# microsoft/vision-longformer

Hardware: NVIDIA H100
Metric: images/sec ViL-Small 224x224 training (higher is better)
Workload: dtype bf16

## Files before the change

### vision_longformer_b200/csrc/vil_sm90.cuh

```cuda
#pragma once
#include <cuda_bf16.h>
#include <cuda_fp16.h>
#include <stdint.h>

namespace sm90 {

__device__ __forceinline__ uint32_t smem_u32(const void* p) { return (uint32_t)__cvta_generic_to_shared(p); }

__host__ __device__ constexpr int core_off(int r, int c, int K) { return (((r >> 3) * (K >> 3) + (c >> 3)) << 6) + ((r & 7) << 3) + (c & 7); }

__device__ __forceinline__ uint64_t desc(const void* tile, int K, int k16) {
  const uint32_t a = smem_u32(tile) + k16 * 256;
  uint64_t d = (uint64_t)((a >> 4) & 0x3FFF);
  d |= (uint64_t)(128 >> 4) << 16;
  d |= (uint64_t)(((K >> 3) * 128) >> 4) << 32;
  return d;
}

__device__ __forceinline__ void wg_fence() { asm volatile("wgmma.fence.sync.aligned;" ::: "memory"); }
__device__ __forceinline__ void wg_commit() { asm volatile("wgmma.commit_group.sync.aligned;" ::: "memory"); }
__device__ __forceinline__ void wg_wait0() { asm volatile("wgmma.wait_group.sync.aligned 0;" ::: "memory"); }
__device__ __forceinline__ void fence_proxy_async() { asm volatile("fence.proxy.async.shared::cta;" ::: "memory"); }
template <int R>
__device__ __forceinline__ void reg_fence(float (&d)[R]) {
#pragma unroll
  for (int i = 0; i < R; ++i) asm volatile("" : "+f"(d[i])::"memory");
}

__device__ __forceinline__ void wgmma_ss_bf16_n16(float (&d)[8], uint64_t a, uint64_t b, uint32_t acc) {
  asm volatile(
      "{\n\t.reg .pred p;\n\tsetp.ne.b32 p, %10, 0;\n\t"
      "wgmma.mma_async.sync.aligned.m64n16k16.f32.bf16.bf16 {%0,%1,%2,%3,%4,%5,%6,%7}, %8, %9, p, 1, 1, 0, 0;\n\t}"
      : "+f"(d[0]), "+f"(d[1]), "+f"(d[2]), "+f"(d[3]), "+f"(d[4]), "+f"(d[5]), "+f"(d[6]), "+f"(d[7])
      : "l"(a), "l"(b), "r"(acc));
}
__device__ __forceinline__ void wgmma_rs_bf16_n16(float (&d)[8], const uint32_t (&a)[4], uint64_t b, uint32_t acc) {
  asm volatile(
      "{\n\t.reg .pred p;\n\tsetp.ne.b32 p, %13, 0;\n\t"
      "wgmma.mma_async.sync.aligned.m64n16k16.f32.bf16.bf16 {%0,%1,%2,%3,%4,%5,%6,%7}, {%8,%9,%10,%11}, %12, p, 1, 1, 0;\n\t}"
      : "+f"(d[0]), "+f"(d[1]), "+f"(d[2]), "+f"(d[3]), "+f"(d[4]), "+f"(d[5]), "+f"(d[6]), "+f"(d[7])
      : "r"(a[0]), "r"(a[1]), "r"(a[2]), "r"(a[3]), "l"(b), "r"(acc));
}
__device__ __forceinline__ void wgmma_ss_f16_n16(float (&d)[8], uint64_t a, uint64_t b, uint32_t acc) {
  asm volatile(
      "{\n\t.reg .pred p;\n\tsetp.ne.b32 p, %10, 0;\n\t"
      "wgmma.mma_async.sync.aligned.m64n16k16.f32.f16.f16 {%0,%1,%2,%3,%4,%5,%6,%7}, %8, %9, p, 1, 1, 0, 0;\n\t}"
      : "+f"(d[0]), "+f"(d[1]), "+f"(d[2]), "+f"(d[3]), "+f"(d[4]), "+f"(d[5]), "+f"(d[6]), "+f"(d[7])
      : "l"(a), "l"(b), "r"(acc));
}
__device__ __forceinline__ void wgmma_rs_f16_n16(float (&d)[8], const uint32_t (&a)[4], uint64_t b, uint32_t acc) {
  asm volatile(
      "{\n\t.reg .pred p;\n\tsetp.ne.b32 p, %13, 0;\n\t"
      "wgmma.mma_async.sync.aligned.m64n16k16.f32.f16.f16 {%0,%1,%2,%3,%4,%5,%6,%7}, {%8,%9,%10,%11}, %12, p, 1, 1, 0;\n\t}"
      : "+f"(d[0]), "+f"(d[1]), "+f"(d[2]), "+f"(d[3]), "+f"(d[4]), "+f"(d[5]), "+f"(d[6]), "+f"(d[7])
      : "r"(a[0]), "r"(a[1]), "r"(a[2]), "r"(a[3]), "l"(b), "r"(acc));
}
__device__ __forceinline__ void wgmma_ss_bf16_n32(float (&d)[16], uint64_t a, uint64_t b, uint32_t acc) {
  asm volatile(
      "{\n\t.reg .pred p;\n\tsetp.ne.b32 p, %18, 0;\n\t"
      "wgmma.mma_async.sync.aligned.m64n32k16.f32.bf16.bf16 {%0,%1,%2,%3,%4,%5,%6,%7,%8,%9,%10,%11,%12,%13,%14,%15}, %16, %17, p, 1, 1, 0, 0;\n\t}"
      : "+f"(d[0]), "+f"(d[1]), "+f"(d[2]), "+f"(d[3]), "+f"(d[4]), "+f"(d[5]), "+f"(d[6]), "+f"(d[7]), "+f"(d[8]), "+f"(d[9]), "+f"(d[10]), "+f"(d[11]), "+f"(d[12]), "+f"(d[13]), "+f"(d[14]), "+f"(d[15])
      : "l"(a), "l"(b), "r"(acc));
}
__device__ __forceinline__ void wgmma_rs_bf16_n32(float (&d)[16], const uint32_t (&a)[4], uint64_t b, uint32_t acc) {
  asm volatile(
      "{\n\t.reg .pred p;\n\tsetp.ne.b32 p, %21, 0;\n\t"
      "wgmma.mma_async.sync.aligned.m64n32k16.f32.bf16.bf16 {%0,%1,%2,%3,%4,%5,%6,%7,%8,%9,%10,%11,%12,%13,%14,%15}, {%16,%17,%18,%19}, %20, p, 1, 1, 0;\n\t}"
      : "+f"(d[0]), "+f"(d[1]), "+f"(d[2]), "+f"(d[3]), "+f"(d[4]), "+f"(d[5]), "+f"(d[6]), "+f"(d[7]), "+f"(d[8]), "+f"(d[9]), "+f"(d[10]), "+f"(d[11]), "+f"(d[12]), "+f"(d[13]), "+f"(d[14]), "+f"(d[15])
      : "r"(a[0]), "r"(a[1]), "r"(a[2]), "r"(a[3]), "l"(b), "r"(acc));
}
__device__ __forceinline__ void wgmma_ss_f16_n32(float (&d)[16], uint64_t a, uint64_t b, uint32_t acc) {
  asm volatile(
      "{\n\t.reg .pred p;\n\tsetp.ne.b32 p, %18, 0;\n\t"
      "wgmma.mma_async.sync.aligned.m64n32k16.f32.f16.f16 {%0,%1,%2,%3,%4,%5,%6,%7,%8,%9,%10,%11,%12,%13,%14,%15}, %16, %17, p, 1, 1, 0, 0;\n\t}"
      : "+f"(d[0]), "+f"(d[1]), "+f"(d[2]), "+f"(d[3]), "+f"(d[4]), "+f"(d[5]), "+f"(d[6]), "+f"(d[7]), "+f"(d[8]), "+f"(d[9]), "+f"(d[10]), "+f"(d[11]), "+f"(d[12]), "+f"(d[13]), "+f"(d[14]), "+f"(d[15])
      : "l"(a), "l"(b), "r"(acc));
}
__device__ __forceinline__ void wgmma_rs_f16_n32(float (&d)[16], const uint32_t (&a)[4], uint64_t b, uint32_t acc) {
  asm volatile(
      "{\n\t.reg .pred p;\n\tsetp.ne.b32 p, %21, 0;\n\t"
      "wgmma.mma_async.sync.aligned.m64n32k16.f32.f16.f16 {%0,%1,%2,%3,%4,%5,%6,%7,%8,%9,%10,%11,%12,%13,%14,%15}, {%16,%17,%18,%19}, %20, p, 1, 1, 0;\n\t}"
      : "+f"(d[0]), "+f"(d[1]), "+f"(d[2]), "+f"(d[3]), "+f"(d[4]), "+f"(d[5]), "+f"(d[6]), "+f"(d[7]), "+f"(d[8]), "+f"(d[9]), "+f"(d[10]), "+f"(d[11]), "+f"(d[12]), "+f"(d[13]), "+f"(d[14]), "+f"(d[15])
      : "r"(a[0]), "r"(a[1]), "r"(a[2]), "r"(a[3]), "l"(b), "r"(acc));
}
__device__ __forceinline__ void wgmma_ss_bf16_n64(float (&d)[32], uint64_t a, uint64_t b, uint32_t acc) {
  asm volatile(
      "{\n\t.reg .pred p;\n\tsetp.ne.b32 p, %34, 0;\n\t"
      "wgmma.mma_async.sync.aligned.m64n64k16.f32.bf16.bf16 {%0,%1,%2,%3,%4,%5,%6,%7,%8,%9,%10,%11,%12,%13,%14,%15,%16,%17,%18,%19,%20,%21,%22,%23,%24,%25,%26,%27,%28,%29,%30,%31}, %32, %33, p, 1, 1, 0, 0;\n\t}"
      : "+f"(d[0]), "+f"(d[1]), "+f"(d[2]), "+f"(d[3]), "+f"(d[4]), "+f"(d[5]), "+f"(d[6]), "+f"(d[7]), "+f"(d[8]), "+f"(d[9]), "+f"(d[10]), "+f"(d[11]), "+f"(d[12]), "+f"(d[13]), "+f"(d[14]), "+f"(d[15]), "+f"(d[16]), "+f"(d[17]), "+f"(d[18]), "+f"(d[19]), "+f"(d[20]), "+f"(d[21]), "+f"(d[22]), "+f"(d[23]), "+f"(d[24]), "+f"(d[25]), "+f"(d[26]), "+f"(d[27]), "+f"(d[28]), "+f"(d[29]), "+f"(d[30]), "+f"(d[31])
      : "l"(a), "l"(b), "r"(acc));
}
__device__ __forceinline__ void wgmma_rs_bf16_n64(float (&d)[32], const uint32_t (&a)[4], uint64_t b, uint32_t acc) {
  asm volatile(
      "{\n\t.reg .pred p;\n\tsetp.ne.b32 p, %37, 0;\n\t"
      "wgmma.mma_async.sync.aligned.m64n64k16.f32.bf16.bf16 {%0,%1,%2,%3,%4,%5,%6,%7,%8,%9,%10,%11,%12,%13,%14,%15,%16,%17,%18,%19,%20,%21,%22,%23,%24,%25,%26,%27,%28,%29,%30,%31}, {%32,%33,%34,%35}, %36, p, 1, 1, 0;\n\t}"
      : "+f"(d[0]), "+f"(d[1]), "+f"(d[2]), "+f"(d[3]), "+f"(d[4]), "+f"(d[5]), "+f"(d[6]), "+f"(d[7]), "+f"(d[8]), "+f"(d[9]), "+f"(d[10]), "+f"(d[11]), "+f"(d[12]), "+f"(d[13]), "+f"(d[14]), "+f"(d[15]), "+f"(d[16]), "+f"(d[17]), "+f"(d[18]), "+f"(d[19]), "+f"(d[20]), "+f"(d[21]), "+f"(d[22]), "+f"(d[23]), "+f"(d[24]), "+f"(d[25]), "+f"(d[26]), "+f"(d[27]), "+f"(d[28]), "+f"(d[29]), "+f"(d[30]), "+f"(d[31])
      : "r"(a[0]), "r"(a[1]), "r"(a[2]), "r"(a[3]), "l"(b), "r"(acc));
}
__device__ __forceinline__ void wgmma_ss_f16_n64(float (&d)[32], uint64_t a, uint64_t b, uint32_t acc) {
  asm volatile(
      "{\n\t.reg .pred p;\n\tsetp.ne.b32 p, %34, 0;\n\t"
      "wgmma.mma_async.sync.aligned.m64n64k16.f32.f16.f16 {%0,%1,%2,%3,%4,%5,%6,%7,%8,%9,%10,%11,%12,%13,%14,%15,%16,%17,%18,%19,%20,%21,%22,%23,%24,%25,%26,%27,%28,%29,%30,%31}, %32, %33, p, 1, 1, 0, 0;\n\t}"
      : "+f"(d[0]), "+f"(d[1]), "+f"(d[2]), "+f"(d[3]), "+f"(d[4]), "+f"(d[5]), "+f"(d[6]), "+f"(d[7]), "+f"(d[8]), "+f"(d[9]), "+f"(d[10]), "+f"(d[11]), "+f"(d[12]), "+f"(d[13]), "+f"(d[14]), "+f"(d[15]), "+f"(d[16]), "+f"(d[17]), "+f"(d[18]), "+f"(d[19]), "+f"(d[20]), "+f"(d[21]), "+f"(d[22]), "+f"(d[23]), "+f"(d[24]), "+f"(d[25]), "+f"(d[26]), "+f"(d[27]), "+f"(d[28]), "+f"(d[29]), "+f"(d[30]), "+f"(d[31])
      : "l"(a), "l"(b), "r"(acc));
}
__device__ __forceinline__ void wgmma_rs_f16_n64(float (&d)[32], const uint32_t (&a)[4], uint64_t b, uint32_t acc) {
  asm volatile(
      "{\n\t.reg .pred p;\n\tsetp.ne.b32 p, %37, 0;\n\t"
      "wgmma.mma_async.sync.aligned.m64n64k16.f32.f16.f16 {%0,%1,%2,%3,%4,%5,%6,%7,%8,%9,%10,%11,%12,%13,%14,%15,%16,%17,%18,%19,%20,%21,%22,%23,%24,%25,%26,%27,%28,%29,%30,%31}, {%32,%33,%34,%35}, %36, p, 1, 1, 0;\n\t}"
      : "+f"(d[0]), "+f"(d[1]), "+f"(d[2]), "+f"(d[3]), "+f"(d[4]), "+f"(d[5]), "+f"(d[6]), "+f"(d[7]), "+f"(d[8]), "+f"(d[9]), "+f"(d[10]), "+f"(d[11]), "+f"(d[12]), "+f"(d[13]), "+f"(d[14]), "+f"(d[15]), "+f"(d[16]), "+f"(d[17]), "+f"(d[18]), "+f"(d[19]), "+f"(d[20]), "+f"(d[21]), "+f"(d[22]), "+f"(d[23]), "+f"(d[24]), "+f"(d[25]), "+f"(d[26]), "+f"(d[27]), "+f"(d[28]), "+f"(d[29]), "+f"(d[30]), "+f"(d[31])
      : "r"(a[0]), "r"(a[1]), "r"(a[2]), "r"(a[3]), "l"(b), "r"(acc));
}

template <typename T, int N> struct Wg;
#define VIL_WG(T, TN, N)                                                                                          \
  template <> struct Wg<T, N> {                                                                                   \
    static __device__ __forceinline__ void ss(float (&d)[N / 2], uint64_t a, uint64_t b, uint32_t acc) { wgmma_ss_##TN##_n##N(d, a, b, acc); } \
    static __device__ __forceinline__ void rs(float (&d)[N / 2], const uint32_t (&a)[4], uint64_t b, uint32_t acc) { wgmma_rs_##TN##_n##N(d, a, b, acc); } \
  };
VIL_WG(__nv_bfloat16, bf16, 16)
VIL_WG(__nv_bfloat16, bf16, 32)
VIL_WG(__nv_bfloat16, bf16, 64)
VIL_WG(__half, f16, 16)
VIL_WG(__half, f16, 32)
VIL_WG(__half, f16, 64)
#undef VIL_WG

template <typename T> __device__ __forceinline__ uint32_t pack2(float x, float y);
template <> __device__ __forceinline__ uint32_t pack2<__nv_bfloat16>(float x, float y) {
  __nv_bfloat162 v = __floats2bfloat162_rn(x, y);
  return *reinterpret_cast<uint32_t*>(&v);
}
template <> __device__ __forceinline__ uint32_t pack2<__half>(float x, float y) {
  __half2 v = __floats2half2_rn(x, y);
  return *reinterpret_cast<uint32_t*>(&v);
}

}
```

### vision_longformer_b200/csrc/vil_wgmma.cu

```cuda
#include <cstdio>
#include "vil_host.cuh"
#include "vil_wgmma.cuh"

namespace vil {
namespace {

int head_tile(int D) { return D <= 16 ? 16 : D <= 32 ? 32 : 64; }
int table_floats(const Geo& g) { return g.has_bias ? (4 * g.w - 1) * (4 * g.w - 1) : 0; }

template <typename K>
int set_smem(K kernel, size_t bytes) {
  if (bytes > 227 * 1024) return shared_fail(VIL_E_UNSUPPORTED, "configuration needs more than 227 KB of shared memory");
  cudaError_t e = cudaFuncSetAttribute(kernel, cudaFuncAttributeMaxDynamicSharedMemorySize, (int)bytes);
  if (e != cudaSuccess) return shared_fail(VIL_E_CUDA, cudaGetErrorString(e));
  return VIL_OK;
}

const char* why_not(const VilAttnParams* p, const Geo& g) {
  if (p->dtype != VIL_BF16 && p->dtype != VIL_F16) return "dtype is fp32 (wgmma operands are bf16 / fp16)";
  if (g.D > 64) return "head dim > 64";
  if (wg::DkvSmem<64>::total(table_floats(g)) > 227 * 1024) return "bias table does not fit in shared memory";
  return nullptr;
}

long long blocks(const Geo& g) { return (long long)g.B * g.H * g.mx * g.my * g.npc; }

template <typename T, int HD, typename TO, bool DROP>
int forward_t(const VilAttnParams* p, const Geo& g, cudaStream_t s) {
  int rc;
  if (!(p->skip_mask & 2)) {
    const size_t sm = wg::FwdSmem<HD>::total(table_floats(g));
    if ((rc = set_smem(wg::wg_fwd_local<T, HD, TO, DROP>, sm))) return rc;
    wg::wg_fwd_local<T, HD, TO, DROP><<<(unsigned)blocks(g), wg::kThreads, sm, s>>>(g, t4(p->q), t4(p->k), t4(p->v), t4(p->o), p->lse,
                                                                            p->bias_table, p->g2l);
    count_launch();
    if ((rc = launch_check("wgmma_fwd_local"))) return rc;
  }
  if (g.g > 0 && !(p->skip_mask & 1)) return simt_global_fwd(p, g, s);
  return VIL_OK;
}

template <typename T, int HD, typename TO, bool DROP>
int backward_t(const VilAttnParams* p, const Geo& g, cudaStream_t s) {
  int rc;
  if (!(p->skip_mask & 8) && (rc = simt_delta(p, g, s))) return rc;
  float* delta = static_cast<float*>(p->workspace);
  const int tabn = table_floats(g);
  if (!(p->skip_mask & 2)) {
    const size_t sm = wg::DqSmem<HD>::total(tabn);
    if ((rc = set_smem(wg::wg_bwd_dq<T, HD, TO, DROP>, sm))) return rc;
    wg::wg_bwd_dq<T, HD, TO, DROP><<<(unsigned)blocks(g), wg::kThreads, sm, s>>>(g, t4(p->q), t4(p->k), t4(p->v), t4(p->d_o), t4(p->dq),
                                                                         p->lse, delta, p->bias_table, p->g2l, p->d_bias_table);
    count_launch();
    if ((rc = launch_check("wgmma_bwd_dq"))) return rc;
  }
  if (!(p->skip_mask & 4)) {
    const size_t sm = wg::DkvSmem<HD>::total(tabn, DROP);
    if ((rc = set_smem(wg::wg_bwd_dkv<T, HD, TO, DROP>, sm))) return rc;
    wg::wg_bwd_dkv<T, HD, TO, DROP><<<(unsigned)blocks(g), wg::kThreads, sm, s>>>(g, t4(p->q), t4(p->k), t4(p->v), t4(p->d_o), t4(p->dk),
                                                                          t4(p->dv), p->lse, delta, p->bias_table);
    count_launch();
    if ((rc = launch_check("wgmma_bwd_dkv"))) return rc;
  }
  if (g.g > 0 && !(p->skip_mask & 1)) return simt_global_bwd(p, g, s, g.N);
  return VIL_OK;
}

template <typename T, typename TO, bool DROP>
int dispatch_hd_drop(const VilAttnParams* p, const Geo& g, cudaStream_t s, bool bwd) {
  switch (head_tile(g.D)) {
    case 16: return bwd ? backward_t<T, 16, TO, DROP>(p, g, s) : forward_t<T, 16, TO, DROP>(p, g, s);
    case 32: return bwd ? backward_t<T, 32, TO, DROP>(p, g, s) : forward_t<T, 32, TO, DROP>(p, g, s);
    default: return bwd ? backward_t<T, 64, TO, DROP>(p, g, s) : forward_t<T, 64, TO, DROP>(p, g, s);
  }
}

template <typename T, typename TO>
int dispatch_hd(const VilAttnParams* p, const Geo& g, cudaStream_t s, bool bwd) {
  return g.drop_p > 0.f ? dispatch_hd_drop<T, TO, true>(p, g, s, bwd) : dispatch_hd_drop<T, TO, false>(p, g, s, bwd);
}

int run(const VilAttnParams* p, const Geo& g, cudaStream_t s, bool bwd) {
  note_kernel(bwd ? "wgmma_bwd" : "wgmma_fwd");
  if (p->dtype == VIL_BF16)
    return out_f32(p) ? dispatch_hd<__nv_bfloat16, float>(p, g, s, bwd) : dispatch_hd<__nv_bfloat16, __nv_bfloat16>(p, g, s, bwd);
  return out_f32(p) ? dispatch_hd<__half, float>(p, g, s, bwd) : dispatch_hd<__half, __half>(p, g, s, bwd);
}

}

const char* tc_why_not(const VilAttnParams* p, const Geo& g, bool) {
  const char* w = why_not(p, g);
  return w ? w : "supported";
}
int tc_supported(const VilAttnParams* p, const Geo& g, bool) { return why_not(p, g) == nullptr; }
int tc_forward(const VilAttnParams* p, const Geo& g, cudaStream_t s) { return run(p, g, s, false); }
int tc_backward(const VilAttnParams* p, const Geo& g, cudaStream_t s) { return run(p, g, s, true); }

}
```

### vision_longformer_b200/csrc/vil_wgmma.cuh

```cuda
#pragma once
#include "vil_common.cuh"
#include "vil_sm90.cuh"

namespace vil {
namespace wg {

constexpr int kThreads = 128;

struct Cta { int b, h, R, C, piece; };

__device__ __forceinline__ Cta decode(const Geo& g, int bid) {
  Cta c;
  c.piece = bid % g.npc; bid /= g.npc;
  c.C = bid % g.my; bid /= g.my;
  c.R = bid % g.mx; bid /= g.mx;
  c.h = bid % g.H;
  c.b = bid / g.H;
  return c;
}

__device__ __forceinline__ int acc_row(int i) { return ((threadIdx.x >> 5) << 4) + ((threadIdx.x & 31) >> 2) + (((i >> 1) & 1) << 3); }
__device__ __forceinline__ int acc_col(int i) { return ((i >> 2) << 3) + ((threadIdx.x & 3) << 1) + (i & 1); }

template <typename T, int HD>
__device__ __forceinline__ void stage_half_row(T* tile, T* tile_t, const float (&x)[HD / 2], int row, int half) {
  constexpr int HH = HD / 2;
#pragma unroll
  for (int g8 = 0; g8 < HH / 8; ++g8) {
    uint4 u;
    u.x = sm90::pack2<T>(x[g8 * 8 + 0], x[g8 * 8 + 1]);
    u.y = sm90::pack2<T>(x[g8 * 8 + 2], x[g8 * 8 + 3]);
    u.z = sm90::pack2<T>(x[g8 * 8 + 4], x[g8 * 8 + 5]);
    u.w = sm90::pack2<T>(x[g8 * 8 + 6], x[g8 * 8 + 7]);
    *reinterpret_cast<uint4*>(tile + sm90::core_off(row, half * HH + g8 * 8, HD)) = u;
  }
  if (tile_t != nullptr) {
#pragma unroll
    for (int i = 0; i < HH; ++i) tile_t[sm90::core_off(half * HH + i, row, 64)] = ElemTraits<T>::from_f(x[i]);
  }
}

template <typename T>
__device__ __forceinline__ void to_a_frag(const float (&s)[32], int kk, uint32_t (&a)[4]) {
  a[0] = sm90::pack2<T>(s[8 * kk + 0], s[8 * kk + 1]);
  a[1] = sm90::pack2<T>(s[8 * kk + 2], s[8 * kk + 3]);
  a[2] = sm90::pack2<T>(s[8 * kk + 4], s[8 * kk + 5]);
  a[3] = sm90::pack2<T>(s[8 * kk + 6], s[8 * kk + 7]);
}

template <typename TO, int HD>
__device__ __forceinline__ void store_rows(const float (&acc)[HD / 2], int e, TO* row, int D, float mul) {
  const int c0 = (threadIdx.x & 3) << 1;
#pragma unroll
  for (int j = 0; j < HD / 8; ++j) {
    const int col = 8 * j + c0;
    if (col < D) row[col] = ElemTraits<TO>::from_f(acc[4 * j + 2 * e] * mul);
    if (col + 1 < D) row[col + 1] = ElemTraits<TO>::from_f(acc[4 * j + 2 * e + 1] * mul);
  }
}

__device__ __forceinline__ void drop_key_piece(float (&x)[32], const Geo& geo, const uint32_t (&row)[2], int cbase, uint32_t sid,
                                               float mul) {
  uint32_t keep = 0;
#pragma unroll 1
  for (int i = 0; i < 32; i += 2) {
    bool k0, k1;
    drop_keep2(geo, (i & 2) ? row[1] : row[0], (uint32_t)(cbase + acc_col(i)), sid, k0, k1);
    keep |= ((uint32_t)k0 | ((uint32_t)k1 << 1)) << i;
  }
#pragma unroll
  for (int i = 0; i < 32; ++i) x[i] = (keep >> i) & 1u ? x[i] * mul : 0.f;
}

__device__ __forceinline__ void drop_rows(const Geo& geo, int R, int C, int piece, uint32_t (&row)[2]) {
#pragma unroll
  for (int e = 0; e < 2; ++e) {
    const int l = piece * 64 + acc_row(2 * e);
    row[e] = (uint32_t)((R * geo.w + l / geo.w) * geo.ny + C * geo.w + l % geo.w);
  }
}

struct Visit {
  int r, c;
  int dR, dC;
  int cut;
  int oi;
};

__device__ __forceinline__ int visit_list(const Geo& geo, int R, int C, int sgn, Visit* vl) {
  int n = 0;
  for (int oi = 0; oi < geo.noffs; ++oi) {
    const int dR = geo.offR[oi], dC = geo.offC[oi];
    int r = R + sgn * dR, c = C + sgn * dC;
    if (geo.exact == -1) { r = (r + geo.mx) % geo.mx; c = (c + geo.my) % geo.my; }
    else if (r < 0 || r >= geo.mx || c < 0 || c >= geo.my) continue;
    const int qR = sgn > 0 ? R : r, qC = sgn > 0 ? C : c;
    if (threadIdx.x == 0) vl[n] = Visit{r, c, dR, dC, (qR + dR == geo.mx - 1) | ((qC + dC == geo.my - 1) << 1), oi};
    ++n;
  }
  return n;
}

__device__ __forceinline__ int drop_col_base(const Geo& geo, const Visit* vl, int ngp, int pi) {
  if (pi < ngp) return pi * 64;
  const int vi = (pi - ngp) / geo.npc;
  return geo.g + vl[vi].oi * geo.w2 + (pi - ngp - vi * geo.npc) * 64;
}

__device__ __forceinline__ void chunk_key(const Geo& geo, const Visit& v, int lk, long long& tok, bool& ok, int& vr, int& vc) {
  const int w = geo.w, kr = lk / w, kc = lk - kr * w;
  const int ar = v.r * w + kr, ac = v.c * w + kc;
  const bool real = (ar < geo.nx) && (ac < geo.ny);
  if (geo.exact == -1)
    ok = !(((v.cut & 1) && (kr >= w - geo.padx)) || ((v.cut & 2) && (kc >= w - geo.pady)));
  else
    ok = real;
  tok = (ok && real) ? geo.g + (long long)ar * geo.ny + ac : -1;
  vr = v.dR * w + kr; vc = v.dC * w + kc;
}

__device__ __forceinline__ void key_slot(const Geo& geo, const Visit* vl, int ngp, int pi, int slot, int& gk, long long& tok,
                                         bool& ok, int& vr, int& vc) {
  gk = -1; tok = -1; ok = false; vr = 0; vc = 0;
  if (pi < ngp) {
    const int t = pi * 64 + slot;
    if (t < geo.g) { gk = t; tok = t; ok = true; }
    return;
  }
  const int vi = (pi - ngp) / geo.npc, lk = (pi - ngp - vi * geo.npc) * 64 + slot;
  if (lk < geo.w2) chunk_key(geo, vl[vi], lk, tok, ok, vr, vc);
}

struct KeyCols {
  float* bias;
  int* tix;
  short* kr;
  short* kc;
};
struct QRows {
  int qr[2], qc[2];
  bool ok[2];
};

__device__ __forceinline__ QRows query_rows(const Geo& geo, int R, int C, int piece) {
  QRows q;
  const int w = geo.w;
#pragma unroll
  for (int e = 0; e < 2; ++e) {
    const int l = piece * 64 + acc_row(2 * e);
    const bool in = l < geo.w2;
    q.qr[e] = in ? l / w : 0; q.qc[e] = in ? l % w : 0;
    q.ok[e] = in && (R * w + q.qr[e] < geo.nx) && (C * w + q.qc[e] < geo.ny);
  }
  return q;
}

__device__ __forceinline__ void stage_key_cols(const Geo& geo, const KeyCols& kc, int h, const float* __restrict__ g2l, int gk,
                                               bool ok, int vr, int vc) {
  const int slot = threadIdx.x >> 1;
  float bias = ok ? 0.f : -INFINITY;
  if (gk >= 0 && geo.has_bias) bias = g2l[((long long)geo.H + h) * geo.g + gk];
  kc.bias[slot] = bias;
  kc.tix[slot] = vr * (4 * geo.w - 1) + vc;
  kc.kr[slot] = (short)vr;
  kc.kc[slot] = (short)vc;
}

__device__ __forceinline__ void row_tix(const Geo& geo, const QRows& q, int (&tb)[2]) {
  const int w = geo.w, tw = 4 * w - 1;
  tb[0] = (q.qr[0] + 2 * w - 1) * tw + q.qc[0] + 2 * w - 1;
  tb[1] = (q.qr[1] + 2 * w - 1) * tw + q.qc[1] + 2 * w - 1;
}

template <bool RPE, bool WIN>
__device__ __forceinline__ float key_score(const Geo& geo, const KeyCols& kc, const float* tab, const QRows& q, const int (&tb)[2],
                                           int e, int j, int gl, float s, int& bidx) {
  float bias = kc.bias[j];
  bidx = -1;
  if (RPE && j >= gl) { bidx = tb[e] - kc.tix[j]; bias += tab[bidx]; }
  if (WIN && (abs(q.qr[e] - kc.kr[j]) > geo.w || abs(q.qc[e] - kc.kc[j]) > geo.w)) return -INFINITY;
  return fmaf(geo.scale, s, bias);
}

__device__ __forceinline__ int key_epilogue(const Geo& geo) { return (geo.has_bias ? 2 : 0) | (geo.exact == 1 ? 1 : 0); }

template <bool RPE, bool WIN>
__device__ __forceinline__ void fwd_scores(float (&s)[32], float (&mx)[2], const Geo& geo, const KeyCols& kc, const float* tab,
                                           const QRows& q, int gl) {
  int tb[2] = {0, 0};
  if (RPE) row_tix(geo, q, tb);
#pragma unroll
  for (int i = 0; i < 32; ++i) {
    const int e = (i >> 1) & 1;
    int bidx;
    s[i] = key_score<RPE, WIN>(geo, kc, tab, q, tb, e, acc_col(i), gl, s[i], bidx);
    mx[e] = fmaxf(mx[e], s[i]);
  }
}

template <bool RPE, bool WIN>
__device__ __forceinline__ void dq_scores(float (&s)[32], const float (&dp)[32], const Geo& geo, const KeyCols& kc,
                                          const float* tab, const QRows& q, int gl, const float (&lse_r)[2],
                                          const float (&del_r)[2], float* __restrict__ d_table, int h) {
  int tb[2] = {0, 0};
  if (RPE) row_tix(geo, q, tb);
#pragma unroll
  for (int i = 0; i < 32; ++i) {
    const int e = (i >> 1) & 1;
    int bidx;
    const float val = key_score<RPE, WIN>(geo, kc, tab, q, tb, e, acc_col(i), gl, s[i], bidx);
    const float ds = __expf(val - lse_r[e]) * (dp[i] - del_r[e]);
    if (RPE && d_table != nullptr && bidx >= 0 && q.ok[e] && val != -INFINITY)
      atomicAdd(d_table + (long long)bidx * geo.H + h, ds);
    s[i] = ds;
  }
}

constexpr size_t kKeyMeta = 64 * (4 + 4 + 2 + 2) + 9 * sizeof(Visit);
constexpr size_t kQueryMeta = 64 * (4 + 4 + 4 + 2 + 2 + 1) + 9 * sizeof(Visit);

__device__ __forceinline__ KeyCols key_cols(float* base, Visit*& vl) {
  KeyCols kc;
  kc.bias = base;
  kc.tix = reinterpret_cast<int*>(kc.bias + 64);
  vl = reinterpret_cast<Visit*>(kc.tix + 64);
  kc.kr = reinterpret_cast<short*>(vl + 9);
  kc.kc = kc.kr + 64;
  return kc;
}

template <int HD> struct FwdSmem {
  static constexpr size_t tiles = 3 * 64 * HD * 2;
  static size_t total(int tabn) { return (tiles + (size_t)tabn * 4 + kKeyMeta + 15) & ~size_t(15); }
};
template <int HD> struct DqSmem {
  static constexpr size_t tiles = 5 * 64 * HD * 2;
  static size_t total(int tabn) { return (tiles + (size_t)tabn * 4 + kKeyMeta + 15) & ~size_t(15); }
};
template <int HD> struct DkvSmem {
  static constexpr size_t tiles = 6 * 64 * HD * 2;
  static size_t total(int tabn, bool drop = false) {
    return (tiles + (size_t)tabn * 4 + kQueryMeta + (drop ? 64 * sizeof(int) : 0) + 15) & ~size_t(15);
  }
};

template <typename T, int HD, typename TO, bool DROP = false>
__global__ void __launch_bounds__(kThreads, HD <= 32 ? 5 : 3)
wg_fwd_local(Geo geo, T4 q, T4 k, T4 v, T4 o, float* __restrict__ lse, const float* __restrict__ table,
             const float* __restrict__ g2l) {
  constexpr int HH = HD / 2;
  using W64 = sm90::Wg<T, 64>;
  using WHD = sm90::Wg<T, HD>;
  extern __shared__ __align__(128) unsigned char smem_raw[];
  T* Qs = reinterpret_cast<T*>(smem_raw);
  T* Ks = Qs + 64 * HD;
  T* Vt = Ks + 64 * HD;
  float* tab = reinterpret_cast<float*>(Vt + 64 * HD);
  const int tabn = geo.has_bias ? (4 * geo.w - 1) * (4 * geo.w - 1) : 0;
  Visit* vl;
  const KeyCols kcol = key_cols(tab + tabn, vl);

  const Cta cid = decode(geo, blockIdx.x);
  const int b = cid.b, h = cid.h, R = cid.R, C = cid.C;
  const int tid = threadIdx.x, slot = tid >> 1, half = tid & 1;
  const int w = geo.w, D = geo.D;
  for (int i = tid; i < tabn; i += kThreads) tab[i] = table[(long long)i * geo.H + h];
  {
    const int l = cid.piece * 64 + slot;
    const int r = R * w + l / w, c = C * w + l % w;
    float x[HH];
#pragma unroll
    for (int i = 0; i < HH; ++i) x[i] = 0.f;
    if (l < geo.w2 && r < geo.nx && c < geo.ny) load_seg<T, HH>(row_ptr<T>(q, b, h, (long long)r * geo.ny + c), half * HH, D, x);
    stage_half_row<T, HD>(Qs, nullptr, x, slot, half);
  }
  float m[2] = {-INFINITY, -INFINITY}, lsum[2] = {0.f, 0.f};
  float oacc[HH];
#pragma unroll
  for (int i = 0; i < HH; ++i) oacc[i] = 0.f;

  const int ngp = (geo.g + 63) / 64, npieces = ngp + visit_list(geo, R, C, 1, vl) * geo.npc;
  const int epi = key_epilogue(geo);
  for (int pi = 0; pi < npieces; ++pi) {
    __syncthreads();
    {
      int gk, vr, vc;
      long long tok;
      bool ok;
      key_slot(geo, vl, ngp, pi, slot, gk, tok, ok, vr, vc);
      float kk[HH], vv[HH];
#pragma unroll
      for (int i = 0; i < HH; ++i) { kk[i] = 0.f; vv[i] = 0.f; }
      if (tok >= 0) {
        load_seg<T, HH>(row_ptr<T>(k, b, h, tok), half * HH, D, kk);
        load_seg<T, HH>(row_ptr<T>(v, b, h, tok), half * HH, D, vv);
      }
      stage_half_row<T, HD>(Ks, nullptr, kk, slot, half);
#pragma unroll
      for (int i = 0; i < HH; ++i) Vt[sm90::core_off(half * HH + i, slot, 64)] = ElemTraits<T>::from_f(vv[i]);
      if (half == 0) stage_key_cols(geo, kcol, h, g2l, gk, ok, vr, vc);
    }
    sm90::fence_proxy_async();
    __syncthreads();
    float s[32];
    sm90::wg_fence();
#pragma unroll
    for (int kk = 0; kk < HD / 16; ++kk) W64::ss(s, sm90::desc(Qs, HD, kk), sm90::desc(Ks, HD, kk), kk > 0);
    sm90::wg_commit();
    sm90::wg_wait0();
    sm90::reg_fence(s);
    float mx[2] = {-INFINITY, -INFINITY};
    const int gl = geo.g - pi * 64;
    switch (epi) {
      case 0: fwd_scores<false, false>(s, mx, geo, kcol, tab, query_rows(geo, R, C, cid.piece), gl); break;
      case 1: fwd_scores<false, true>(s, mx, geo, kcol, tab, query_rows(geo, R, C, cid.piece), gl); break;
      case 2: fwd_scores<true, false>(s, mx, geo, kcol, tab, query_rows(geo, R, C, cid.piece), gl); break;
      default: fwd_scores<true, true>(s, mx, geo, kcol, tab, query_rows(geo, R, C, cid.piece), gl); break;
    }
    float corr[2];
#pragma unroll
    for (int e = 0; e < 2; ++e) {
      mx[e] = fmaxf(mx[e], __shfl_xor_sync(0xffffffffu, mx[e], 1));
      mx[e] = fmaxf(mx[e], __shfl_xor_sync(0xffffffffu, mx[e], 2));
      const float mn = fmaxf(m[e], mx[e]);
      corr[e] = (mn == -INFINITY) ? 1.f : __expf(m[e] - mn);
      m[e] = mn;
      lsum[e] *= corr[e];
    }
#pragma unroll
    for (int i = 0; i < 32; ++i) {
      const int e = (i >> 1) & 1;
      const float p = (m[e] == -INFINITY) ? 0.f : __expf(s[i] - m[e]);
      s[i] = p;
      lsum[e] += p;
    }
#pragma unroll
    for (int i = 0; i < HH; ++i) oacc[i] *= corr[(i >> 1) & 1];
    if constexpr (DROP) {
      uint32_t drow[2];
      drop_rows(geo, R, C, cid.piece, drow);
      drop_key_piece(s, geo, drow, drop_col_base(geo, vl, ngp, pi), 2u * (uint32_t)(b * geo.H + h), 1.f);
    }
    uint32_t a[4][4];
#pragma unroll
    for (int kk = 0; kk < 4; ++kk) to_a_frag<T>(s, kk, a[kk]);
    sm90::wg_fence();
#pragma unroll
    for (int kk = 0; kk < 4; ++kk) WHD::rs(oacc, a[kk], sm90::desc(Vt, 64, kk), 1);
    sm90::wg_commit();
    sm90::wg_wait0();
    sm90::reg_fence(oacc);
  }
  const QRows qrow = query_rows(geo, R, C, cid.piece);
#pragma unroll
  for (int e = 0; e < 2; ++e) {
    lsum[e] += __shfl_xor_sync(0xffffffffu, lsum[e], 1);
    lsum[e] += __shfl_xor_sync(0xffffffffu, lsum[e], 2);
    if (!qrow.ok[e]) continue;
    const long long tokq = (long long)(R * w + qrow.qr[e]) * geo.ny + (C * w + qrow.qc[e]);
    const float inv = lsum[e] > 0.f ? 1.f / lsum[e] : 0.f;
    store_rows<TO, HD>(oacc, e, row_ptr_w<TO>(o, b, h, tokq), D, DROP ? inv * geo.drop_scale : inv);
    if ((tid & 3) == 0) lse[((long long)b * geo.H + h) * geo.Nloc + tokq] = m[e] + logf(lsum[e]);
  }
}

template <typename T, int HD, typename TO, bool DROP = false>
__global__ void __launch_bounds__(kThreads)
wg_bwd_dq(Geo geo, T4 q, T4 k, T4 v, T4 d_o, T4 dq, const float* __restrict__ lse, const float* __restrict__ delta,
          const float* __restrict__ table, const float* __restrict__ g2l, float* __restrict__ d_table) {
  constexpr int HH = HD / 2;
  using W64 = sm90::Wg<T, 64>;
  using WHD = sm90::Wg<T, HD>;
  extern __shared__ __align__(128) unsigned char smem_raw[];
  T* Qs = reinterpret_cast<T*>(smem_raw);
  T* Gs = Qs + 64 * HD;
  T* Ks = Gs + 64 * HD;
  T* Vs = Ks + 64 * HD;
  T* Kt = Vs + 64 * HD;
  float* tab = reinterpret_cast<float*>(Kt + 64 * HD);
  const int tabn = geo.has_bias ? (4 * geo.w - 1) * (4 * geo.w - 1) : 0;
  Visit* vl;
  const KeyCols kcol = key_cols(tab + tabn, vl);

  const Cta cid = decode(geo, blockIdx.x);
  const int b = cid.b, h = cid.h, R = cid.R, C = cid.C;
  const int tid = threadIdx.x, slot = tid >> 1, half = tid & 1;
  const int w = geo.w, D = geo.D;
  const long long bh = (long long)b * geo.H + h;
  for (int i = tid; i < tabn; i += kThreads) tab[i] = table[(long long)i * geo.H + h];
  {
    const int l = cid.piece * 64 + slot;
    const int r = R * w + l / w, c = C * w + l % w;
    float x[HH], y[HH];
#pragma unroll
    for (int i = 0; i < HH; ++i) { x[i] = 0.f; y[i] = 0.f; }
    if (l < geo.w2 && r < geo.nx && c < geo.ny) {
      load_seg<T, HH>(row_ptr<T>(q, b, h, (long long)r * geo.ny + c), half * HH, D, x);
      load_seg<T, HH>(row_ptr<T>(d_o, b, h, (long long)r * geo.ny + c), half * HH, D, y);
    }
    stage_half_row<T, HD>(Qs, nullptr, x, slot, half);
    stage_half_row<T, HD>(Gs, nullptr, y, slot, half);
  }
  const QRows qrow = query_rows(geo, R, C, cid.piece);
  float lse_r[2], del_r[2];
#pragma unroll
  for (int e = 0; e < 2; ++e) {
    lse_r[e] = INFINITY; del_r[e] = 0.f;
    if (qrow.ok[e]) {
      const long long tokq = (long long)(R * w + qrow.qr[e]) * geo.ny + (C * w + qrow.qc[e]);
      lse_r[e] = lse[bh * geo.Nloc + tokq];
      del_r[e] = delta[bh * geo.Nloc + tokq];
    }
  }
  float dqacc[HH];
#pragma unroll
  for (int i = 0; i < HH; ++i) dqacc[i] = 0.f;

  const int ngp = (geo.g + 63) / 64, npieces = ngp + visit_list(geo, R, C, 1, vl) * geo.npc;
  const int epi = key_epilogue(geo);
  for (int pi = 0; pi < npieces; ++pi) {
    __syncthreads();
    {
      int gk, vr, vc;
      long long tok;
      bool ok;
      key_slot(geo, vl, ngp, pi, slot, gk, tok, ok, vr, vc);
      float kk[HH], vv[HH];
#pragma unroll
      for (int i = 0; i < HH; ++i) { kk[i] = 0.f; vv[i] = 0.f; }
      if (tok >= 0) {
        load_seg<T, HH>(row_ptr<T>(k, b, h, tok), half * HH, D, kk);
        load_seg<T, HH>(row_ptr<T>(v, b, h, tok), half * HH, D, vv);
      }
      stage_half_row<T, HD>(Ks, Kt, kk, slot, half);
      stage_half_row<T, HD>(Vs, nullptr, vv, slot, half);
      if (half == 0) stage_key_cols(geo, kcol, h, g2l, gk, ok, vr, vc);
    }
    sm90::fence_proxy_async();
    __syncthreads();
    float s[32], dp[32];
    sm90::wg_fence();
#pragma unroll
    for (int kk = 0; kk < HD / 16; ++kk) W64::ss(s, sm90::desc(Qs, HD, kk), sm90::desc(Ks, HD, kk), kk > 0);
#pragma unroll
    for (int kk = 0; kk < HD / 16; ++kk) W64::ss(dp, sm90::desc(Gs, HD, kk), sm90::desc(Vs, HD, kk), kk > 0);
    sm90::wg_commit();
    sm90::wg_wait0();
    sm90::reg_fence(s);
    sm90::reg_fence(dp);
    const int gl = geo.g - pi * 64;
    if constexpr (DROP) {
      uint32_t drow[2];
      drop_rows(geo, R, C, cid.piece, drow);
      drop_key_piece(dp, geo, drow, drop_col_base(geo, vl, ngp, pi), 2u * (uint32_t)(b * geo.H + h), geo.drop_scale);
    }
    switch (epi) {
      case 0: dq_scores<false, false>(s, dp, geo, kcol, tab, qrow, gl, lse_r, del_r, d_table, h); break;
      case 1: dq_scores<false, true>(s, dp, geo, kcol, tab, qrow, gl, lse_r, del_r, d_table, h); break;
      case 2: dq_scores<true, false>(s, dp, geo, kcol, tab, qrow, gl, lse_r, del_r, d_table, h); break;
      default: dq_scores<true, true>(s, dp, geo, kcol, tab, qrow, gl, lse_r, del_r, d_table, h); break;
    }
    uint32_t a[4][4];
#pragma unroll
    for (int kk = 0; kk < 4; ++kk) to_a_frag<T>(s, kk, a[kk]);
    sm90::wg_fence();
#pragma unroll
    for (int kk = 0; kk < 4; ++kk) WHD::rs(dqacc, a[kk], sm90::desc(Kt, 64, kk), 1);
    sm90::wg_commit();
    sm90::wg_wait0();
    sm90::reg_fence(dqacc);
  }
#pragma unroll
  for (int e = 0; e < 2; ++e) {
    if (!qrow.ok[e]) continue;
    const long long tokq = (long long)(R * w + qrow.qr[e]) * geo.ny + (C * w + qrow.qc[e]);
    store_rows<TO, HD>(dqacc, e, row_ptr_w<TO>(dq, b, h, tokq), D, geo.scale);
  }
}


struct QueryCols {
  float* lse;
  float* del;
  int* tix;
  short* qr;
  short* qc;
  unsigned char* cut;
  int* tok;
};
struct KRows {
  int kr[2], kc[2], tb[2];
  int cut[2];
  bool real[2];
};

__device__ __forceinline__ QueryCols query_cols(float* base, Visit*& vl) {
  QueryCols qc;
  qc.lse = base;
  qc.del = qc.lse + 64;
  qc.tix = reinterpret_cast<int*>(qc.del + 64);
  vl = reinterpret_cast<Visit*>(qc.tix + 64);
  qc.qr = reinterpret_cast<short*>(vl + 9);
  qc.qc = qc.qr + 64;
  qc.cut = reinterpret_cast<unsigned char*>(qc.qc + 64);
  qc.tok = reinterpret_cast<int*>(qc.cut + 64);
  return qc;
}

__device__ __forceinline__ int query_epilogue(const Geo& geo) {
  return (geo.has_bias ? 3 : 0) + (geo.exact == 1 ? 1 : geo.exact == -1 ? 2 : 0);
}

template <bool RPE, int MASK>
__device__ __forceinline__ void dkv_probs(float (&s)[32], float (&dp)[32], const Geo& geo, const QueryCols& qc, const float* tab,
                                          const KRows& kr) {
#pragma unroll
  for (int i = 0; i < 32; ++i) {
    const int e = (i >> 1) & 1, j = acc_col(i);
    float x = fmaf(geo.scale, s[i], RPE ? tab[qc.tix[j] - kr.tb[e]] : 0.f) - qc.lse[j];
    if (MASK == 1 && (abs(qc.qr[j] - kr.kr[e]) > geo.w || abs(qc.qc[j] - kr.kc[e]) > geo.w)) x = -INFINITY;
    if (MASK == 2 && (qc.cut[j] & kr.cut[e])) x = -INFINITY;
    const float p = __expf(x);
    s[i] = p;
    dp[i] = p * (dp[i] - qc.del[j]);
  }
}

template <typename T, int HD, typename TO, bool DROP = false>
__global__ void __launch_bounds__(kThreads)
wg_bwd_dkv(Geo geo, T4 q, T4 k, T4 v, T4 d_o, T4 dk, T4 dv, const float* __restrict__ lse, const float* __restrict__ delta,
           const float* __restrict__ table) {
  constexpr int HH = HD / 2;
  using W64 = sm90::Wg<T, 64>;
  using WHD = sm90::Wg<T, HD>;
  extern __shared__ __align__(128) unsigned char smem_raw[];
  T* Ks = reinterpret_cast<T*>(smem_raw);
  T* Vs = Ks + 64 * HD;
  T* Qs = Vs + 64 * HD;
  T* Gs = Qs + 64 * HD;
  T* Qt = Gs + 64 * HD;
  T* Gt = Qt + 64 * HD;
  float* tab = reinterpret_cast<float*>(Gt + 64 * HD);
  const int tw = 4 * geo.w - 1;
  const int tabn = geo.has_bias ? tw * tw : 0;
  Visit* vl;
  const QueryCols qcol = query_cols(tab + tabn, vl);

  const Cta cid = decode(geo, blockIdx.x);
  const int b = cid.b, h = cid.h, KR = cid.R, KC = cid.C;
  const int tid = threadIdx.x, slot = tid >> 1, half = tid & 1;
  const int w = geo.w, D = geo.D;
  const long long bh = (long long)b * geo.H + h;
  for (int i = tid; i < tabn; i += kThreads) tab[i] = table[(long long)i * geo.H + h];
  {
    const int lk = cid.piece * 64 + slot;
    const int ar = KR * w + lk / w, ac = KC * w + lk % w;
    float x[HH], y[HH];
#pragma unroll
    for (int i = 0; i < HH; ++i) { x[i] = 0.f; y[i] = 0.f; }
    if (lk < geo.w2 && ar < geo.nx && ac < geo.ny) {
      const long long tokk = geo.g + (long long)ar * geo.ny + ac;
      load_seg<T, HH>(row_ptr<T>(k, b, h, tokk), half * HH, D, x);
      load_seg<T, HH>(row_ptr<T>(v, b, h, tokk), half * HH, D, y);
    }
    stage_half_row<T, HD>(Ks, nullptr, x, slot, half);
    stage_half_row<T, HD>(Vs, nullptr, y, slot, half);
  }
  KRows krow;
#pragma unroll
  for (int e = 0; e < 2; ++e) {
    const int lk = cid.piece * 64 + acc_row(2 * e);
    const bool in = lk < geo.w2;
    krow.kr[e] = in ? lk / w : 0; krow.kc[e] = in ? lk % w : 0;
    krow.real[e] = in && (KR * w + krow.kr[e] < geo.nx) && (KC * w + krow.kc[e] < geo.ny);
    krow.tb[e] = krow.kr[e] * tw + krow.kc[e] - (2 * w - 1) * (tw + 1);
    krow.cut[e] = (krow.kr[e] >= w - geo.padx) | ((krow.kc[e] >= w - geo.pady) << 1);
  }
  float dkacc[HH], dvacc[HH];
#pragma unroll
  for (int i = 0; i < HH; ++i) { dkacc[i] = 0.f; dvacc[i] = 0.f; }

  const int npieces = visit_list(geo, KR, KC, -1, vl) * geo.npc;
  const int epi = query_epilogue(geo);
  for (int qp = 0; qp < npieces; ++qp) {
    __syncthreads();
    {
      const int vi = qp / geo.npc, l = (qp - vi * geo.npc) * 64 + slot;
      bool qv = false;
      long long tq = 0;
      int qa = 0, qb = 0, cut = 0;
      if (l < geo.w2) {
        const int qrr = l / w, qcc = l - qrr * w;
        const Visit vq = vl[vi];
        const int r = vq.r * w + qrr, c = vq.c * w + qcc;
        qv = (r < geo.nx) && (c < geo.ny);
        tq = (long long)r * geo.ny + c;
        qa = qrr - vq.dR * w; qb = qcc - vq.dC * w; cut = vq.cut;
      }
      float x[HH], y[HH];
#pragma unroll
      for (int i = 0; i < HH; ++i) { x[i] = 0.f; y[i] = 0.f; }
      if (qv) {
        load_seg<T, HH>(row_ptr<T>(q, b, h, tq), half * HH, D, x);
        load_seg<T, HH>(row_ptr<T>(d_o, b, h, tq), half * HH, D, y);
      }
      stage_half_row<T, HD>(Qs, Qt, x, slot, half);
      stage_half_row<T, HD>(Gs, Gt, y, slot, half);
      if (half == 0) {
        qcol.lse[slot] = qv ? lse[bh * geo.Nloc + tq] : INFINITY;
        qcol.del[slot] = qv ? delta[bh * geo.Nloc + tq] : 0.f;
        qcol.tix[slot] = qa * tw + qb;
        qcol.qr[slot] = (short)qa; qcol.qc[slot] = (short)qb;
        qcol.cut[slot] = (unsigned char)cut;
        if (DROP) qcol.tok[slot] = (int)tq;
      }
    }
    sm90::fence_proxy_async();
    __syncthreads();
    float s[32], dp[32];
    sm90::wg_fence();
#pragma unroll
    for (int kk = 0; kk < HD / 16; ++kk) W64::ss(s, sm90::desc(Ks, HD, kk), sm90::desc(Qs, HD, kk), kk > 0);
#pragma unroll
    for (int kk = 0; kk < HD / 16; ++kk) W64::ss(dp, sm90::desc(Vs, HD, kk), sm90::desc(Gs, HD, kk), kk > 0);
    sm90::wg_commit();
    sm90::wg_wait0();
    sm90::reg_fence(s);
    sm90::reg_fence(dp);
    uint32_t keep = 0;
    if constexpr (DROP) {
      const int vi = qp / geo.npc;
      const uint32_t c0 = (uint32_t)(geo.g + vl[vi].oi * geo.w2 + cid.piece * 64), sid = 2u * (uint32_t)(b * geo.H + h);
#pragma unroll 1
      for (int i = 0; i < 32; ++i)
        keep |= (uint32_t)drop_keep(geo, (uint32_t)qcol.tok[acc_col(i)], c0 + (uint32_t)acc_row(i), sid) << i;
#pragma unroll
      for (int i = 0; i < 32; ++i) dp[i] = (keep >> i) & 1u ? dp[i] * geo.drop_scale : 0.f;
    }
    switch (epi) {
      case 0: dkv_probs<false, 0>(s, dp, geo, qcol, tab, krow); break;
      case 1: dkv_probs<false, 1>(s, dp, geo, qcol, tab, krow); break;
      case 2: dkv_probs<false, 2>(s, dp, geo, qcol, tab, krow); break;
      case 3: dkv_probs<true, 0>(s, dp, geo, qcol, tab, krow); break;
      case 4: dkv_probs<true, 1>(s, dp, geo, qcol, tab, krow); break;
      default: dkv_probs<true, 2>(s, dp, geo, qcol, tab, krow); break;
    }
    if constexpr (DROP) {
#pragma unroll
      for (int i = 0; i < 32; ++i) s[i] = (keep >> i) & 1u ? s[i] * geo.drop_scale : 0.f;
    }
    uint32_t ap[4][4], ad[4][4];
#pragma unroll
    for (int kk = 0; kk < 4; ++kk) { to_a_frag<T>(s, kk, ap[kk]); to_a_frag<T>(dp, kk, ad[kk]); }
    sm90::wg_fence();
#pragma unroll
    for (int kk = 0; kk < 4; ++kk) WHD::rs(dvacc, ap[kk], sm90::desc(Gt, 64, kk), 1);
#pragma unroll
    for (int kk = 0; kk < 4; ++kk) WHD::rs(dkacc, ad[kk], sm90::desc(Qt, 64, kk), 1);
    sm90::wg_commit();
    sm90::wg_wait0();
    sm90::reg_fence(dvacc);
    sm90::reg_fence(dkacc);
  }
#pragma unroll
  for (int e = 0; e < 2; ++e) {
    if (!krow.real[e]) continue;
    const long long tokk = geo.g + (long long)(KR * w + krow.kr[e]) * geo.ny + (KC * w + krow.kc[e]);
    store_rows<TO, HD>(dkacc, e, row_ptr_w<TO>(dk, b, h, tokk), D, geo.scale);
    store_rows<TO, HD>(dvacc, e, row_ptr_w<TO>(dv, b, h, tokk), D, 1.f);
  }
}

}
}
```

Before: 3635.

## Pipeline K/V and Q/dO staging with cp.async ring buffers in attention kernels

Replaces the synchronous register load, convert and store of each key/value or query/grad-output piece with a three-stage cp.async ring buffer. The next pieces' global loads now overlap the current piece's wgmma work. The explicitly transposed Q/dO tiles are dropped; the second GEMMs read the same tiles through transposed (MN-major) wgmma descriptors. The cost is more shared memory per CTA, which lowers occupancy, plus a new 16-byte alignment requirement that sends misaligned inputs to the fallback path.

```diff
diff --git a/vision_longformer_b200/csrc/vil_sm90.cuh b/vision_longformer_b200/csrc/vil_sm90.cuh
--- a/vision_longformer_b200/csrc/vil_sm90.cuh
+++ b/vision_longformer_b200/csrc/vil_sm90.cuh
@@ -9,13 +9,25 @@
 
 __host__ __device__ constexpr int core_off(int r, int c, int K) { return (((r >> 3) * (K >> 3) + (c >> 3)) << 6) + ((r & 7) << 3) + (c & 7); }
 
+__device__ __forceinline__ uint64_t make_desc(uint32_t addr, uint32_t lbo, uint32_t sbo) {
+  return (uint64_t)((addr >> 4) & 0x3FFF) | (uint64_t)(lbo >> 4) << 16 | (uint64_t)(sbo >> 4) << 32;
+}
 __device__ __forceinline__ uint64_t desc(const void* tile, int K, int k16) {
-  const uint32_t a = smem_u32(tile) + k16 * 256;
-  uint64_t d = (uint64_t)((a >> 4) & 0x3FFF);
-  d |= (uint64_t)(128 >> 4) << 16;
-  d |= (uint64_t)(((K >> 3) * 128) >> 4) << 32;
-  return d;
+  return make_desc(smem_u32(tile) + k16 * 256, 128, (K >> 3) * 128);
 }
+__device__ __forceinline__ uint64_t desc_mn(const void* tile, int N, int k16) {
+  return make_desc(smem_u32(tile) + k16 * N * 32, N * 16, 128);
+}
+
+__device__ __forceinline__ void cp_async16(void* dst, const void* src, int n) {
+  asm volatile("cp.async.cg.shared.global [%0], [%1], 16, %2;" ::"r"(smem_u32(dst)), "l"(src), "r"(n) : "memory");
+}
+__device__ __forceinline__ void cp_async4(void* dst, const void* src) {
+  asm volatile("cp.async.ca.shared.global [%0], [%1], 4;" ::"r"(smem_u32(dst)), "l"(src) : "memory");
+}
+__device__ __forceinline__ void cp_async_commit() { asm volatile("cp.async.commit_group;" ::: "memory"); }
+template <int N>
+__device__ __forceinline__ void cp_async_wait() { asm volatile("cp.async.wait_group %0;" ::"n"(N) : "memory"); }
 
 __device__ __forceinline__ void wg_fence() { asm volatile("wgmma.fence.sync.aligned;" ::: "memory"); }
 __device__ __forceinline__ void wg_commit() { asm volatile("wgmma.commit_group.sync.aligned;" ::: "memory"); }
@@ -37,7 +49,7 @@
 __device__ __forceinline__ void wgmma_rs_bf16_n16(float (&d)[8], const uint32_t (&a)[4], uint64_t b, uint32_t acc) {
   asm volatile(
       "{\n\t.reg .pred p;\n\tsetp.ne.b32 p, %13, 0;\n\t"
-      "wgmma.mma_async.sync.aligned.m64n16k16.f32.bf16.bf16 {%0,%1,%2,%3,%4,%5,%6,%7}, {%8,%9,%10,%11}, %12, p, 1, 1, 0;\n\t}"
+      "wgmma.mma_async.sync.aligned.m64n16k16.f32.bf16.bf16 {%0,%1,%2,%3,%4,%5,%6,%7}, {%8,%9,%10,%11}, %12, p, 1, 1, 1;\n\t}"
       : "+f"(d[0]), "+f"(d[1]), "+f"(d[2]), "+f"(d[3]), "+f"(d[4]), "+f"(d[5]), "+f"(d[6]), "+f"(d[7])
       : "r"(a[0]), "r"(a[1]), "r"(a[2]), "r"(a[3]), "l"(b), "r"(acc));
 }
@@ -51,7 +63,7 @@
 __device__ __forceinline__ void wgmma_rs_f16_n16(float (&d)[8], const uint32_t (&a)[4], uint64_t b, uint32_t acc) {
   asm volatile(
       "{\n\t.reg .pred p;\n\tsetp.ne.b32 p, %13, 0;\n\t"
-      "wgmma.mma_async.sync.aligned.m64n16k16.f32.f16.f16 {%0,%1,%2,%3,%4,%5,%6,%7}, {%8,%9,%10,%11}, %12, p, 1, 1, 0;\n\t}"
+      "wgmma.mma_async.sync.aligned.m64n16k16.f32.f16.f16 {%0,%1,%2,%3,%4,%5,%6,%7}, {%8,%9,%10,%11}, %12, p, 1, 1, 1;\n\t}"
       : "+f"(d[0]), "+f"(d[1]), "+f"(d[2]), "+f"(d[3]), "+f"(d[4]), "+f"(d[5]), "+f"(d[6]), "+f"(d[7])
       : "r"(a[0]), "r"(a[1]), "r"(a[2]), "r"(a[3]), "l"(b), "r"(acc));
 }
@@ -65,7 +77,7 @@
 __device__ __forceinline__ void wgmma_rs_bf16_n32(float (&d)[16], const uint32_t (&a)[4], uint64_t b, uint32_t acc) {
   asm volatile(
       "{\n\t.reg .pred p;\n\tsetp.ne.b32 p, %21, 0;\n\t"
-      "wgmma.mma_async.sync.aligned.m64n32k16.f32.bf16.bf16 {%0,%1,%2,%3,%4,%5,%6,%7,%8,%9,%10,%11,%12,%13,%14,%15}, {%16,%17,%18,%19}, %20, p, 1, 1, 0;\n\t}"
+      "wgmma.mma_async.sync.aligned.m64n32k16.f32.bf16.bf16 {%0,%1,%2,%3,%4,%5,%6,%7,%8,%9,%10,%11,%12,%13,%14,%15}, {%16,%17,%18,%19}, %20, p, 1, 1, 1;\n\t}"
       : "+f"(d[0]), "+f"(d[1]), "+f"(d[2]), "+f"(d[3]), "+f"(d[4]), "+f"(d[5]), "+f"(d[6]), "+f"(d[7]), "+f"(d[8]), "+f"(d[9]), "+f"(d[10]), "+f"(d[11]), "+f"(d[12]), "+f"(d[13]), "+f"(d[14]), "+f"(d[15])
       : "r"(a[0]), "r"(a[1]), "r"(a[2]), "r"(a[3]), "l"(b), "r"(acc));
 }
@@ -79,7 +91,7 @@
 __device__ __forceinline__ void wgmma_rs_f16_n32(float (&d)[16], const uint32_t (&a)[4], uint64_t b, uint32_t acc) {
   asm volatile(
       "{\n\t.reg .pred p;\n\tsetp.ne.b32 p, %21, 0;\n\t"
-      "wgmma.mma_async.sync.aligned.m64n32k16.f32.f16.f16 {%0,%1,%2,%3,%4,%5,%6,%7,%8,%9,%10,%11,%12,%13,%14,%15}, {%16,%17,%18,%19}, %20, p, 1, 1, 0;\n\t}"
+      "wgmma.mma_async.sync.aligned.m64n32k16.f32.f16.f16 {%0,%1,%2,%3,%4,%5,%6,%7,%8,%9,%10,%11,%12,%13,%14,%15}, {%16,%17,%18,%19}, %20, p, 1, 1, 1;\n\t}"
       : "+f"(d[0]), "+f"(d[1]), "+f"(d[2]), "+f"(d[3]), "+f"(d[4]), "+f"(d[5]), "+f"(d[6]), "+f"(d[7]), "+f"(d[8]), "+f"(d[9]), "+f"(d[10]), "+f"(d[11]), "+f"(d[12]), "+f"(d[13]), "+f"(d[14]), "+f"(d[15])
       : "r"(a[0]), "r"(a[1]), "r"(a[2]), "r"(a[3]), "l"(b), "r"(acc));
 }
@@ -93,7 +105,7 @@
 __device__ __forceinline__ void wgmma_rs_bf16_n64(float (&d)[32], const uint32_t (&a)[4], uint64_t b, uint32_t acc) {
   asm volatile(
       "{\n\t.reg .pred p;\n\tsetp.ne.b32 p, %37, 0;\n\t"
-      "wgmma.mma_async.sync.aligned.m64n64k16.f32.bf16.bf16 {%0,%1,%2,%3,%4,%5,%6,%7,%8,%9,%10,%11,%12,%13,%14,%15,%16,%17,%18,%19,%20,%21,%22,%23,%24,%25,%26,%27,%28,%29,%30,%31}, {%32,%33,%34,%35}, %36, p, 1, 1, 0;\n\t}"
+      "wgmma.mma_async.sync.aligned.m64n64k16.f32.bf16.bf16 {%0,%1,%2,%3,%4,%5,%6,%7,%8,%9,%10,%11,%12,%13,%14,%15,%16,%17,%18,%19,%20,%21,%22,%23,%24,%25,%26,%27,%28,%29,%30,%31}, {%32,%33,%34,%35}, %36, p, 1, 1, 1;\n\t}"
       : "+f"(d[0]), "+f"(d[1]), "+f"(d[2]), "+f"(d[3]), "+f"(d[4]), "+f"(d[5]), "+f"(d[6]), "+f"(d[7]), "+f"(d[8]), "+f"(d[9]), "+f"(d[10]), "+f"(d[11]), "+f"(d[12]), "+f"(d[13]), "+f"(d[14]), "+f"(d[15]), "+f"(d[16]), "+f"(d[17]), "+f"(d[18]), "+f"(d[19]), "+f"(d[20]), "+f"(d[21]), "+f"(d[22]), "+f"(d[23]), "+f"(d[24]), "+f"(d[25]), "+f"(d[26]), "+f"(d[27]), "+f"(d[28]), "+f"(d[29]), "+f"(d[30]), "+f"(d[31])
       : "r"(a[0]), "r"(a[1]), "r"(a[2]), "r"(a[3]), "l"(b), "r"(acc));
 }
@@ -107,7 +119,7 @@
 __device__ __forceinline__ void wgmma_rs_f16_n64(float (&d)[32], const uint32_t (&a)[4], uint64_t b, uint32_t acc) {
   asm volatile(
       "{\n\t.reg .pred p;\n\tsetp.ne.b32 p, %37, 0;\n\t"
-      "wgmma.mma_async.sync.aligned.m64n64k16.f32.f16.f16 {%0,%1,%2,%3,%4,%5,%6,%7,%8,%9,%10,%11,%12,%13,%14,%15,%16,%17,%18,%19,%20,%21,%22,%23,%24,%25,%26,%27,%28,%29,%30,%31}, {%32,%33,%34,%35}, %36, p, 1, 1, 0;\n\t}"
+      "wgmma.mma_async.sync.aligned.m64n64k16.f32.f16.f16 {%0,%1,%2,%3,%4,%5,%6,%7,%8,%9,%10,%11,%12,%13,%14,%15,%16,%17,%18,%19,%20,%21,%22,%23,%24,%25,%26,%27,%28,%29,%30,%31}, {%32,%33,%34,%35}, %36, p, 1, 1, 1;\n\t}"
       : "+f"(d[0]), "+f"(d[1]), "+f"(d[2]), "+f"(d[3]), "+f"(d[4]), "+f"(d[5]), "+f"(d[6]), "+f"(d[7]), "+f"(d[8]), "+f"(d[9]), "+f"(d[10]), "+f"(d[11]), "+f"(d[12]), "+f"(d[13]), "+f"(d[14]), "+f"(d[15]), "+f"(d[16]), "+f"(d[17]), "+f"(d[18]), "+f"(d[19]), "+f"(d[20]), "+f"(d[21]), "+f"(d[22]), "+f"(d[23]), "+f"(d[24]), "+f"(d[25]), "+f"(d[26]), "+f"(d[27]), "+f"(d[28]), "+f"(d[29]), "+f"(d[30]), "+f"(d[31])
       : "r"(a[0]), "r"(a[1]), "r"(a[2]), "r"(a[3]), "l"(b), "r"(acc));
 }
diff --git a/vision_longformer_b200/csrc/vil_wgmma.cu b/vision_longformer_b200/csrc/vil_wgmma.cu
--- a/vision_longformer_b200/csrc/vil_wgmma.cu
+++ b/vision_longformer_b200/csrc/vil_wgmma.cu
@@ -16,9 +16,16 @@
   return VIL_OK;
 }
 
-const char* why_not(const VilAttnParams* p, const Geo& g) {
+bool rows_aligned16(const VilTensor4& t) {
+  constexpr long long e = 2;
+  return reinterpret_cast<uintptr_t>(t.ptr) % 16 == 0 && (t.sb * e) % 16 == 0 && (t.sh * e) % 16 == 0 && (t.st * e) % 16 == 0;
+}
+
+const char* why_not(const VilAttnParams* p, const Geo& g, bool bwd) {
   if (p->dtype != VIL_BF16 && p->dtype != VIL_F16) return "dtype is fp32 (wgmma operands are bf16 / fp16)";
   if (g.D > 64) return "head dim > 64";
+  if (g.D % 8 != 0 || !rows_aligned16(p->q) || !rows_aligned16(p->k) || !rows_aligned16(p->v) || (bwd && !rows_aligned16(p->d_o)))
+    return "q / k / v / d_o rows are not 16-byte aligned (D % 8 != 0, or a pointer or b / h / t stride off 16 bytes)";
   if (wg::DkvSmem<64>::total(table_floats(g)) > 227 * 1024) return "bias table does not fit in shared memory";
   return nullptr;
 }
@@ -89,11 +96,11 @@
 
 }
 
-const char* tc_why_not(const VilAttnParams* p, const Geo& g, bool) {
-  const char* w = why_not(p, g);
+const char* tc_why_not(const VilAttnParams* p, const Geo& g, bool bwd) {
+  const char* w = why_not(p, g, bwd);
   return w ? w : "supported";
 }
-int tc_supported(const VilAttnParams* p, const Geo& g, bool) { return why_not(p, g) == nullptr; }
+int tc_supported(const VilAttnParams* p, const Geo& g, bool bwd) { return why_not(p, g, bwd) == nullptr; }
 int tc_forward(const VilAttnParams* p, const Geo& g, cudaStream_t s) { return run(p, g, s, false); }
 int tc_backward(const VilAttnParams* p, const Geo& g, cudaStream_t s) { return run(p, g, s, true); }
 
diff --git a/vision_longformer_b200/csrc/vil_wgmma.cuh b/vision_longformer_b200/csrc/vil_wgmma.cuh
--- a/vision_longformer_b200/csrc/vil_wgmma.cuh
+++ b/vision_longformer_b200/csrc/vil_wgmma.cuh
@@ -22,21 +22,17 @@
 __device__ __forceinline__ int acc_row(int i) { return ((threadIdx.x >> 5) << 4) + ((threadIdx.x & 31) >> 2) + (((i >> 1) & 1) << 3); }
 __device__ __forceinline__ int acc_col(int i) { return ((i >> 2) << 3) + ((threadIdx.x & 3) << 1) + (i & 1); }
 
+constexpr int kStages = 3;
+
 template <typename T, int HD>
-__device__ __forceinline__ void stage_half_row(T* tile, T* tile_t, const float (&x)[HD / 2], int row, int half) {
+__device__ __forceinline__ void stage_row(T* tile, const T* base, long long st, long long tok, int row, int half, int D) {
   constexpr int HH = HD / 2;
+  const T* src = base + (tok < 0 ? 0 : tok * st);
 #pragma unroll
   for (int g8 = 0; g8 < HH / 8; ++g8) {
-    uint4 u;
-    u.x = sm90::pack2<T>(x[g8 * 8 + 0], x[g8 * 8 + 1]);
-    u.y = sm90::pack2<T>(x[g8 * 8 + 2], x[g8 * 8 + 3]);
-    u.z = sm90::pack2<T>(x[g8 * 8 + 4], x[g8 * 8 + 5]);
-    u.w = sm90::pack2<T>(x[g8 * 8 + 6], x[g8 * 8 + 7]);
-    *reinterpret_cast<uint4*>(tile + sm90::core_off(row, half * HH + g8 * 8, HD)) = u;
-  }
-  if (tile_t != nullptr) {
-#pragma unroll
-    for (int i = 0; i < HH; ++i) tile_t[sm90::core_off(half * HH + i, row, 64)] = ElemTraits<T>::from_f(x[i]);
+    const int c = half * HH + g8 * 8;
+    const bool in = tok >= 0 && c < D;
+    sm90::cp_async16(tile + sm90::core_off(row, c, HD), in ? src + c : base, in ? 16 : 0);
   }
 }
 
@@ -107,8 +103,20 @@
   return geo.g + vl[vi].oi * geo.w2 + (pi - ngp - vi * geo.npc) * 64;
 }
 
-__device__ __forceinline__ void chunk_key(const Geo& geo, const Visit& v, int lk, long long& tok, bool& ok, int& vr, int& vc) {
-  const int w = geo.w, kr = lk / w, kc = lk - kr * w;
+struct SlotWalk {
+  int vi, pj, kr, kc;
+  int r0, c0, dr, dc;
+  __device__ __forceinline__ SlotWalk(const Geo& geo, int slot)
+      : vi(0), pj(0), r0(slot / geo.w), c0(slot % geo.w), dr(64 / geo.w), dc(64 % geo.w) { kr = r0; kc = c0; }
+  __device__ __forceinline__ void next(const Geo& geo) {
+    if (++pj == geo.npc) { pj = 0; ++vi; kr = r0; kc = c0; return; }
+    kr += dr; kc += dc;
+    if (kc >= geo.w) { kc -= geo.w; ++kr; }
+  }
+};
+
+__device__ __forceinline__ void chunk_key(const Geo& geo, const Visit& v, int kr, int kc, long long& tok, bool& ok, int& vr, int& vc) {
+  const int w = geo.w;
   const int ar = v.r * w + kr, ac = v.c * w + kc;
   const bool real = (ar < geo.nx) && (ac < geo.ny);
   if (geo.exact == -1)
@@ -119,16 +127,16 @@
   vr = v.dR * w + kr; vc = v.dC * w + kc;
 }
 
-__device__ __forceinline__ void key_slot(const Geo& geo, const Visit* vl, int ngp, int pi, int slot, int& gk, long long& tok,
-                                         bool& ok, int& vr, int& vc) {
+__device__ __forceinline__ void key_slot(const Geo& geo, const Visit* vl, int ngp, int pi, int slot, SlotWalk& wk, int& gk,
+                                         long long& tok, bool& ok, int& vr, int& vc) {
   gk = -1; tok = -1; ok = false; vr = 0; vc = 0;
   if (pi < ngp) {
     const int t = pi * 64 + slot;
     if (t < geo.g) { gk = t; tok = t; ok = true; }
     return;
   }
-  const int vi = (pi - ngp) / geo.npc, lk = (pi - ngp - vi * geo.npc) * 64 + slot;
-  if (lk < geo.w2) chunk_key(geo, vl[vi], lk, tok, ok, vr, vc);
+  if (wk.kr < geo.w) chunk_key(geo, vl[wk.vi], wk.kr, wk.kc, tok, ok, vr, vc);
+  wk.next(geo);
 }
 
 struct KeyCols {
@@ -216,49 +224,73 @@
   }
 }
 
-constexpr size_t kKeyMeta = 64 * (4 + 4 + 2 + 2) + 9 * sizeof(Visit);
-constexpr size_t kQueryMeta = 64 * (4 + 4 + 4 + 2 + 2 + 1) + 9 * sizeof(Visit);
-
-__device__ __forceinline__ KeyCols key_cols(float* base, Visit*& vl) {
+constexpr size_t kKeyCols = 64 * (4 + 4 + 2 + 2);
+constexpr size_t kQueryCols = 64 * (4 + 4 + 4 + 2 + 2 + 1);
+constexpr size_t kVisits = 9 * sizeof(Visit);
+__host__ __device__ constexpr size_t query_cols_bytes(bool drop) { return kQueryCols + (drop ? 64 * sizeof(int) : 0); }
+
+__device__ __forceinline__ KeyCols key_cols(unsigned char* meta, int stage) {
   KeyCols kc;
-  kc.bias = base;
+  kc.bias = reinterpret_cast<float*>(meta + stage * kKeyCols);
   kc.tix = reinterpret_cast<int*>(kc.bias + 64);
-  vl = reinterpret_cast<Visit*>(kc.tix + 64);
-  kc.kr = reinterpret_cast<short*>(vl + 9);
+  kc.kr = reinterpret_cast<short*>(kc.tix + 64);
   kc.kc = kc.kr + 64;
   return kc;
 }
 
 template <int HD> struct FwdSmem {
-  static constexpr size_t tiles = 3 * 64 * HD * 2;
-  static size_t total(int tabn) { return (tiles + (size_t)tabn * 4 + kKeyMeta + 15) & ~size_t(15); }
+  static constexpr size_t tiles = (1 + 2 * kStages) * 64 * HD * 2;
+  static size_t total(int tabn) { return (tiles + kStages * kKeyCols + kVisits + (size_t)tabn * 4 + 15) & ~size_t(15); }
 };
 template <int HD> struct DqSmem {
-  static constexpr size_t tiles = 5 * 64 * HD * 2;
-  static size_t total(int tabn) { return (tiles + (size_t)tabn * 4 + kKeyMeta + 15) & ~size_t(15); }
+  static constexpr size_t tiles = (2 + 2 * kStages) * 64 * HD * 2;
+  static size_t total(int tabn) { return (tiles + kStages * kKeyCols + kVisits + (size_t)tabn * 4 + 15) & ~size_t(15); }
 };
 template <int HD> struct DkvSmem {
-  static constexpr size_t tiles = 6 * 64 * HD * 2;
+  static constexpr size_t tiles = (2 + 2 * kStages) * 64 * HD * 2;
   static size_t total(int tabn, bool drop = false) {
-    return (tiles + (size_t)tabn * 4 + kQueryMeta + (drop ? 64 * sizeof(int) : 0) + 15) & ~size_t(15);
-  }
-};
+    return (tiles + kStages * query_cols_bytes(drop) + kVisits + 64 * sizeof(int) + (size_t)tabn * 4 + 15) & ~size_t(15);
+  }
+};
+
+template <typename T, int HD>
+__device__ __forceinline__ void issue_key_piece(const Geo& geo, int pi, int npieces, int ngp, const Visit* vl, SlotWalk& wk,
+                                                T* ring, unsigned char* meta, const T* kb, long long kst, const T* vb,
+                                                long long vst, int h, const float* __restrict__ g2l) {
+  if (pi < npieces) {
+    const int slot = threadIdx.x >> 1, half = threadIdx.x & 1, st = pi % kStages;
+    int gk, vr, vc;
+    long long tok;
+    bool ok;
+    key_slot(geo, vl, ngp, pi, slot, wk, gk, tok, ok, vr, vc);
+    T* Ks = ring + st * 2 * 64 * HD;
+    stage_row<T, HD>(Ks, kb, kst, tok, slot, half, geo.D);
+    stage_row<T, HD>(Ks + 64 * HD, vb, vst, tok, slot, half, geo.D);
+    if (half == 0) stage_key_cols(geo, key_cols(meta, st), h, g2l, gk, ok, vr, vc);
+  }
+  sm90::cp_async_commit();
+}
+
+__device__ __forceinline__ void ring_wait() {
+  sm90::cp_async_wait<kStages - 2>();
+  sm90::fence_proxy_async();
+  __syncthreads();
+}
 
 template <typename T, int HD, typename TO, bool DROP = false>
 __global__ void __launch_bounds__(kThreads, HD <= 32 ? 5 : 3)
 wg_fwd_local(Geo geo, T4 q, T4 k, T4 v, T4 o, float* __restrict__ lse, const float* __restrict__ table,
              const float* __restrict__ g2l) {
-  constexpr int HH = HD / 2;
+  constexpr int HH = HD / 2, TILE = 64 * HD;
   using W64 = sm90::Wg<T, 64>;
   using WHD = sm90::Wg<T, HD>;
   extern __shared__ __align__(128) unsigned char smem_raw[];
   T* Qs = reinterpret_cast<T*>(smem_raw);
-  T* Ks = Qs + 64 * HD;
-  T* Vt = Ks + 64 * HD;
-  float* tab = reinterpret_cast<float*>(Vt + 64 * HD);
+  T* ring = Qs + TILE;
+  unsigned char* meta = reinterpret_cast<unsigned char*>(ring + 2 * kStages * TILE);
+  Visit* vl = reinterpret_cast<Visit*>(meta + kStages * kKeyCols);
+  float* tab = reinterpret_cast<float*>(vl + 9);
   const int tabn = geo.has_bias ? (4 * geo.w - 1) * (4 * geo.w - 1) : 0;
-  Visit* vl;
-  const KeyCols kcol = key_cols(tab + tabn, vl);
 
   const Cta cid = decode(geo, blockIdx.x);
   const int b = cid.b, h = cid.h, R = cid.R, C = cid.C;
@@ -268,11 +300,8 @@
   {
     const int l = cid.piece * 64 + slot;
     const int r = R * w + l / w, c = C * w + l % w;
-    float x[HH];
-#pragma unroll
-    for (int i = 0; i < HH; ++i) x[i] = 0.f;
-    if (l < geo.w2 && r < geo.nx && c < geo.ny) load_seg<T, HH>(row_ptr<T>(q, b, h, (long long)r * geo.ny + c), half * HH, D, x);
-    stage_half_row<T, HD>(Qs, nullptr, x, slot, half);
+    const bool real = l < geo.w2 && r < geo.nx && c < geo.ny;
+    stage_row<T, HD>(Qs, row_ptr<T>(q, b, h, 0), q.st, real ? (long long)r * geo.ny + c : -1, slot, half, D);
   }
   float m[2] = {-INFINITY, -INFINITY}, lsum[2] = {0.f, 0.f};
   float oacc[HH];
@@ -281,27 +310,20 @@
 
   const int ngp = (geo.g + 63) / 64, npieces = ngp + visit_list(geo, R, C, 1, vl) * geo.npc;
   const int epi = key_epilogue(geo);
+  const T* kb = row_ptr<T>(k, b, h, 0);
+  const T* vb = row_ptr<T>(v, b, h, 0);
+  SlotWalk wk(geo, slot);
+  __syncthreads();
+#pragma unroll
+  for (int p = 0; p < kStages - 1; ++p)
+    issue_key_piece<T, HD>(geo, p, npieces, ngp, vl, wk, ring, meta, kb, k.st, vb, v.st, h, g2l);
   for (int pi = 0; pi < npieces; ++pi) {
-    __syncthreads();
-    {
-      int gk, vr, vc;
-      long long tok;
-      bool ok;
-      key_slot(geo, vl, ngp, pi, slot, gk, tok, ok, vr, vc);
-      float kk[HH], vv[HH];
-#pragma unroll
-      for (int i = 0; i < HH; ++i) { kk[i] = 0.f; vv[i] = 0.f; }
-      if (tok >= 0) {
-        load_seg<T, HH>(row_ptr<T>(k, b, h, tok), half * HH, D, kk);
-        load_seg<T, HH>(row_ptr<T>(v, b, h, tok), half * HH, D, vv);
-      }
-      stage_half_row<T, HD>(Ks, nullptr, kk, slot, half);
-#pragma unroll
-      for (int i = 0; i < HH; ++i) Vt[sm90::core_off(half * HH + i, slot, 64)] = ElemTraits<T>::from_f(vv[i]);
-      if (half == 0) stage_key_cols(geo, kcol, h, g2l, gk, ok, vr, vc);
-    }
-    sm90::fence_proxy_async();
-    __syncthreads();
+    ring_wait();
+    issue_key_piece<T, HD>(geo, pi + kStages - 1, npieces, ngp, vl, wk, ring, meta, kb, k.st, vb, v.st, h, g2l);
+    const int st = pi % kStages;
+    const T* Ks = ring + st * 2 * TILE;
+    const T* Vs = Ks + TILE;
+    const KeyCols kcol = key_cols(meta, st);
     float s[32];
     sm90::wg_fence();
 #pragma unroll
@@ -346,7 +368,7 @@
     for (int kk = 0; kk < 4; ++kk) to_a_frag<T>(s, kk, a[kk]);
     sm90::wg_fence();
 #pragma unroll
-    for (int kk = 0; kk < 4; ++kk) WHD::rs(oacc, a[kk], sm90::desc(Vt, 64, kk), 1);
+    for (int kk = 0; kk < 4; ++kk) WHD::rs(oacc, a[kk], sm90::desc_mn(Vs, HD, kk), 1);
     sm90::wg_commit();
     sm90::wg_wait0();
     sm90::reg_fence(oacc);
@@ -368,19 +390,17 @@
 __global__ void __launch_bounds__(kThreads)
 wg_bwd_dq(Geo geo, T4 q, T4 k, T4 v, T4 d_o, T4 dq, const float* __restrict__ lse, const float* __restrict__ delta,
           const float* __restrict__ table, const float* __restrict__ g2l, float* __restrict__ d_table) {
-  constexpr int HH = HD / 2;
+  constexpr int HH = HD / 2, TILE = 64 * HD;
   using W64 = sm90::Wg<T, 64>;
   using WHD = sm90::Wg<T, HD>;
   extern __shared__ __align__(128) unsigned char smem_raw[];
   T* Qs = reinterpret_cast<T*>(smem_raw);
-  T* Gs = Qs + 64 * HD;
-  T* Ks = Gs + 64 * HD;
-  T* Vs = Ks + 64 * HD;
-  T* Kt = Vs + 64 * HD;
-  float* tab = reinterpret_cast<float*>(Kt + 64 * HD);
+  T* Gs = Qs + TILE;
+  T* ring = Gs + TILE;
+  unsigned char* meta = reinterpret_cast<unsigned char*>(ring + 2 * kStages * TILE);
+  Visit* vl = reinterpret_cast<Visit*>(meta + kStages * kKeyCols);
+  float* tab = reinterpret_cast<float*>(vl + 9);
   const int tabn = geo.has_bias ? (4 * geo.w - 1) * (4 * geo.w - 1) : 0;
-  Visit* vl;
-  const KeyCols kcol = key_cols(tab + tabn, vl);
 
   const Cta cid = decode(geo, blockIdx.x);
   const int b = cid.b, h = cid.h, R = cid.R, C = cid.C;
@@ -391,15 +411,9 @@
   {
     const int l = cid.piece * 64 + slot;
     const int r = R * w + l / w, c = C * w + l % w;
-    float x[HH], y[HH];
-#pragma unroll
-    for (int i = 0; i < HH; ++i) { x[i] = 0.f; y[i] = 0.f; }
-    if (l < geo.w2 && r < geo.nx && c < geo.ny) {
-      load_seg<T, HH>(row_ptr<T>(q, b, h, (long long)r * geo.ny + c), half * HH, D, x);
-      load_seg<T, HH>(row_ptr<T>(d_o, b, h, (long long)r * geo.ny + c), half * HH, D, y);
-    }
-    stage_half_row<T, HD>(Qs, nullptr, x, slot, half);
-    stage_half_row<T, HD>(Gs, nullptr, y, slot, half);
+    const long long tokq = (l < geo.w2 && r < geo.nx && c < geo.ny) ? (long long)r * geo.ny + c : -1;
+    stage_row<T, HD>(Qs, row_ptr<T>(q, b, h, 0), q.st, tokq, slot, half, D);
+    stage_row<T, HD>(Gs, row_ptr<T>(d_o, b, h, 0), d_o.st, tokq, slot, half, D);
   }
   const QRows qrow = query_rows(geo, R, C, cid.piece);
   float lse_r[2], del_r[2];
@@ -418,26 +432,20 @@
 
   const int ngp = (geo.g + 63) / 64, npieces = ngp + visit_list(geo, R, C, 1, vl) * geo.npc;
   const int epi = key_epilogue(geo);
+  const T* kb = row_ptr<T>(k, b, h, 0);
+  const T* vb = row_ptr<T>(v, b, h, 0);
+  SlotWalk wk(geo, slot);
+  __syncthreads();
+#pragma unroll
+  for (int p = 0; p < kStages - 1; ++p)
+    issue_key_piece<T, HD>(geo, p, npieces, ngp, vl, wk, ring, meta, kb, k.st, vb, v.st, h, g2l);
   for (int pi = 0; pi < npieces; ++pi) {
-    __syncthreads();
-    {
-      int gk, vr, vc;
-      long long tok;
-      bool ok;
-      key_slot(geo, vl, ngp, pi, slot, gk, tok, ok, vr, vc);
-      float kk[HH], vv[HH];
-#pragma unroll
-      for (int i = 0; i < HH; ++i) { kk[i] = 0.f; vv[i] = 0.f; }
-      if (tok >= 0) {
-        load_seg<T, HH>(row_ptr<T>(k, b, h, tok), half * HH, D, kk);
-        load_seg<T, HH>(row_ptr<T>(v, b, h, tok), half * HH, D, vv);
-      }
-      stage_half_row<T, HD>(Ks, Kt, kk, slot, half);
-      stage_half_row<T, HD>(Vs, nullptr, vv, slot, half);
-      if (half == 0) stage_key_cols(geo, kcol, h, g2l, gk, ok, vr, vc);
-    }
-    sm90::fence_proxy_async();
-    __syncthreads();
+    ring_wait();
+    issue_key_piece<T, HD>(geo, pi + kStages - 1, npieces, ngp, vl, wk, ring, meta, kb, k.st, vb, v.st, h, g2l);
+    const int st = pi % kStages;
+    const T* Ks = ring + st * 2 * TILE;
+    const T* Vs = Ks + TILE;
+    const KeyCols kcol = key_cols(meta, st);
     float s[32], dp[32];
     sm90::wg_fence();
 #pragma unroll
@@ -465,7 +473,7 @@
     for (int kk = 0; kk < 4; ++kk) to_a_frag<T>(s, kk, a[kk]);
     sm90::wg_fence();
 #pragma unroll
-    for (int kk = 0; kk < 4; ++kk) WHD::rs(dqacc, a[kk], sm90::desc(Kt, 64, kk), 1);
+    for (int kk = 0; kk < 4; ++kk) WHD::rs(dqacc, a[kk], sm90::desc_mn(Ks, HD, kk), 1);
     sm90::wg_commit();
     sm90::wg_wait0();
     sm90::reg_fence(dqacc);
@@ -494,17 +502,75 @@
   bool real[2];
 };
 
-__device__ __forceinline__ QueryCols query_cols(float* base, Visit*& vl) {
+__device__ __forceinline__ int key_pos(const Geo& geo, int piece, int row) {
+  const int lk = piece * 64 + row;
+  return lk < geo.w2 ? (lk / geo.w) | ((lk % geo.w) << 8) | (1 << 16) : 0;
+}
+
+__device__ __forceinline__ KRows key_rows(const Geo& geo, int KR, int KC, const int* kpos) {
+  KRows k;
+  const int w = geo.w, tw = 4 * w - 1;
+#pragma unroll
+  for (int e = 0; e < 2; ++e) {
+    const int pos = kpos[acc_row(2 * e)];
+    const bool in = pos >> 16;
+    k.kr[e] = pos & 0xff; k.kc[e] = (pos >> 8) & 0xff;
+    k.real[e] = in && (KR * w + k.kr[e] < geo.nx) && (KC * w + k.kc[e] < geo.ny);
+    k.tb[e] = k.kr[e] * tw + k.kc[e] - (2 * w - 1) * (tw + 1);
+    k.cut[e] = (k.kr[e] >= w - geo.padx) | ((k.kc[e] >= w - geo.pady) << 1);
+  }
+  return k;
+}
+
+__device__ __forceinline__ QueryCols query_cols(unsigned char* meta, int stage, int bytes) {
   QueryCols qc;
-  qc.lse = base;
+  qc.lse = reinterpret_cast<float*>(meta + stage * bytes);
   qc.del = qc.lse + 64;
   qc.tix = reinterpret_cast<int*>(qc.del + 64);
-  vl = reinterpret_cast<Visit*>(qc.tix + 64);
-  qc.qr = reinterpret_cast<short*>(vl + 9);
+  qc.qr = reinterpret_cast<short*>(qc.tix + 64);
   qc.qc = qc.qr + 64;
   qc.cut = reinterpret_cast<unsigned char*>(qc.qc + 64);
   qc.tok = reinterpret_cast<int*>(qc.cut + 64);
   return qc;
+}
+
+template <typename T, int HD, bool DROP>
+__device__ __forceinline__ void issue_query_piece(const Geo& geo, int qp, int npieces, const Visit* vl, SlotWalk& wk, T* ring,
+                                                  unsigned char* meta, const T* qb, long long qst, const T* gb, long long gst,
+                                                  const float* __restrict__ lse, const float* __restrict__ delta) {
+  if (qp < npieces) {
+    const int slot = threadIdx.x >> 1, half = threadIdx.x & 1, st = qp % kStages, w = geo.w;
+    bool qv = false;
+    long long tq = 0;
+    int qa = 0, qb2 = 0, cut = 0;
+    if (wk.kr < w) {
+      const Visit vq = vl[wk.vi];
+      const int r = vq.r * w + wk.kr, c = vq.c * w + wk.kc;
+      qv = (r < geo.nx) && (c < geo.ny);
+      tq = (long long)r * geo.ny + c;
+      qa = wk.kr - vq.dR * w; qb2 = wk.kc - vq.dC * w; cut = vq.cut;
+    }
+    wk.next(geo);
+    T* Qs = ring + st * 2 * 64 * HD;
+    stage_row<T, HD>(Qs, qb, qst, qv ? tq : -1, slot, half, geo.D);
+    stage_row<T, HD>(Qs + 64 * HD, gb, gst, qv ? tq : -1, slot, half, geo.D);
+    if (half == 0) {
+      const QueryCols qcol = query_cols(meta, st, (int)query_cols_bytes(DROP));
+      if (qv) {
+        sm90::cp_async4(qcol.lse + slot, lse + tq);
+        sm90::cp_async4(qcol.del + slot, delta + tq);
+      } else {
+        qcol.lse[slot] = INFINITY;
+        qcol.del[slot] = 0.f;
+      }
+      const int tw = 4 * w - 1;
+      qcol.tix[slot] = qa * tw + qb2;
+      qcol.qr[slot] = (short)qa; qcol.qc[slot] = (short)qb2;
+      qcol.cut[slot] = (unsigned char)cut;
+      if (DROP) qcol.tok[slot] = (int)tq;
+    }
+  }
+  sm90::cp_async_commit();
 }
 
 __device__ __forceinline__ int query_epilogue(const Geo& geo) {
@@ -527,24 +593,23 @@
 }
 
 template <typename T, int HD, typename TO, bool DROP = false>
-__global__ void __launch_bounds__(kThreads)
+__global__ void __launch_bounds__(kThreads, (HD <= 32 ? 4 : 3) - (DROP ? 1 : 0))
 wg_bwd_dkv(Geo geo, T4 q, T4 k, T4 v, T4 d_o, T4 dk, T4 dv, const float* __restrict__ lse, const float* __restrict__ delta,
            const float* __restrict__ table) {
-  constexpr int HH = HD / 2;
+  constexpr int HH = HD / 2, TILE = 64 * HD;
   using W64 = sm90::Wg<T, 64>;
   using WHD = sm90::Wg<T, HD>;
   extern __shared__ __align__(128) unsigned char smem_raw[];
   T* Ks = reinterpret_cast<T*>(smem_raw);
-  T* Vs = Ks + 64 * HD;
-  T* Qs = Vs + 64 * HD;
-  T* Gs = Qs + 64 * HD;
-  T* Qt = Gs + 64 * HD;
-  T* Gt = Qt + 64 * HD;
-  float* tab = reinterpret_cast<float*>(Gt + 64 * HD);
+  T* Vs = Ks + TILE;
+  T* ring = Vs + TILE;
+  unsigned char* meta = reinterpret_cast<unsigned char*>(ring + 2 * kStages * TILE);
+  const int cols = (int)query_cols_bytes(DROP);
+  Visit* vl = reinterpret_cast<Visit*>(meta + kStages * cols);
+  int* kpos = reinterpret_cast<int*>(vl + 9);
+  float* tab = reinterpret_cast<float*>(kpos + 64);
   const int tw = 4 * geo.w - 1;
   const int tabn = geo.has_bias ? tw * tw : 0;
-  Visit* vl;
-  const QueryCols qcol = query_cols(tab + tabn, vl);
 
   const Cta cid = decode(geo, blockIdx.x);
   const int b = cid.b, h = cid.h, KR = cid.R, KC = cid.C;
@@ -555,26 +620,10 @@
   {
     const int lk = cid.piece * 64 + slot;
     const int ar = KR * w + lk / w, ac = KC * w + lk % w;
-    float x[HH], y[HH];
-#pragma unroll
-    for (int i = 0; i < HH; ++i) { x[i] = 0.f; y[i] = 0.f; }
-    if (lk < geo.w2 && ar < geo.nx && ac < geo.ny) {
-      const long long tokk = geo.g + (long long)ar * geo.ny + ac;
-      load_seg<T, HH>(row_ptr<T>(k, b, h, tokk), half * HH, D, x);
-      load_seg<T, HH>(row_ptr<T>(v, b, h, tokk), half * HH, D, y);
-    }
-    stage_half_row<T, HD>(Ks, nullptr, x, slot, half);
-    stage_half_row<T, HD>(Vs, nullptr, y, slot, half);
-  }
-  KRows krow;
-#pragma unroll
-  for (int e = 0; e < 2; ++e) {
-    const int lk = cid.piece * 64 + acc_row(2 * e);
-    const bool in = lk < geo.w2;
-    krow.kr[e] = in ? lk / w : 0; krow.kc[e] = in ? lk % w : 0;
-    krow.real[e] = in && (KR * w + krow.kr[e] < geo.nx) && (KC * w + krow.kc[e] < geo.ny);
-    krow.tb[e] = krow.kr[e] * tw + krow.kc[e] - (2 * w - 1) * (tw + 1);
-    krow.cut[e] = (krow.kr[e] >= w - geo.padx) | ((krow.kc[e] >= w - geo.pady) << 1);
+    const long long tokk = (lk < geo.w2 && ar < geo.nx && ac < geo.ny) ? geo.g + (long long)ar * geo.ny + ac : -1;
+    stage_row<T, HD>(Ks, row_ptr<T>(k, b, h, 0), k.st, tokk, slot, half, D);
+    stage_row<T, HD>(Vs, row_ptr<T>(v, b, h, 0), v.st, tokk, slot, half, D);
+    if (half == 0) kpos[slot] = key_pos(geo, cid.piece, slot);
   }
   float dkacc[HH], dvacc[HH];
 #pragma unroll
@@ -582,51 +631,20 @@
 
   const int npieces = visit_list(geo, KR, KC, -1, vl) * geo.npc;
   const int epi = query_epilogue(geo);
+  SlotWalk wk(geo, slot);
+  __syncthreads();
+#pragma unroll
+  for (int p = 0; p < kStages - 1; ++p)
+    issue_query_piece<T, HD, DROP>(geo, p, npieces, vl, wk, ring, meta, row_ptr<T>(q, b, h, 0), q.st,
+                                   row_ptr<T>(d_o, b, h, 0), d_o.st, lse + bh * geo.Nloc, delta + bh * geo.Nloc);
   for (int qp = 0; qp < npieces; ++qp) {
-    __syncthreads();
-    {
-      const int vi = qp / geo.npc, l = (qp - vi * geo.npc) * 64 + slot;
-      bool qv = false;
-      long long tq = 0;
-      int qa = 0, qb = 0, cut = 0;
-      if (l < geo.w2) {
-        const int qrr = l / w, qcc = l - qrr * w;
-        const Visit vq = vl[vi];
-        const int r = vq.r * w + qrr, c = vq.c * w + qcc;
-        qv = (r < geo.nx) && (c < geo.ny);
-        tq = (long long)r * geo.ny + c;
-        qa = qrr - vq.dR * w; qb = qcc - vq.dC * w; cut = vq.cut;
-      }
-      float x[HH], y[HH];
-#pragma unroll
-      for (int i = 0; i < HH; ++i) { x[i] = 0.f; y[i] = 0.f; }
-      if (qv) {
-        load_seg<T, HH>(row_ptr<T>(q, b, h, tq), half * HH, D, x);
-        load_seg<T, HH>(row_ptr<T>(d_o, b, h, tq), half * HH, D, y);
-      }
-      stage_half_row<T, HD>(Qs, Qt, x, slot, half);
-      stage_half_row<T, HD>(Gs, Gt, y, slot, half);
-      if (half == 0) {
-        qcol.lse[slot] = qv ? lse[bh * geo.Nloc + tq] : INFINITY;
-        qcol.del[slot] = qv ? delta[bh * geo.Nloc + tq] : 0.f;
-        qcol.tix[slot] = qa * tw + qb;
-        qcol.qr[slot] = (short)qa; qcol.qc[slot] = (short)qb;
-        qcol.cut[slot] = (unsigned char)cut;
-        if (DROP) qcol.tok[slot] = (int)tq;
-      }
-    }
-    sm90::fence_proxy_async();
-    __syncthreads();
-    float s[32], dp[32];
-    sm90::wg_fence();
-#pragma unroll
-    for (int kk = 0; kk < HD / 16; ++kk) W64::ss(s, sm90::desc(Ks, HD, kk), sm90::desc(Qs, HD, kk), kk > 0);
-#pragma unroll
-    for (int kk = 0; kk < HD / 16; ++kk) W64::ss(dp, sm90::desc(Vs, HD, kk), sm90::desc(Gs, HD, kk), kk > 0);
-    sm90::wg_commit();
-    sm90::wg_wait0();
-    sm90::reg_fence(s);
-    sm90::reg_fence(dp);
+    ring_wait();
+    issue_query_piece<T, HD, DROP>(geo, qp + kStages - 1, npieces, vl, wk, ring, meta, row_ptr<T>(q, b, h, 0), q.st,
+                                   row_ptr<T>(d_o, b, h, 0), d_o.st, lse + bh * geo.Nloc, delta + bh * geo.Nloc);
+    const int st = qp % kStages;
+    const T* Qs = ring + st * 2 * TILE;
+    const T* Gs = Qs + TILE;
+    const QueryCols qcol = query_cols(meta, st, cols);
     uint32_t keep = 0;
     if constexpr (DROP) {
       const int vi = qp / geo.npc;
@@ -634,16 +652,28 @@
 #pragma unroll 1
       for (int i = 0; i < 32; ++i)
         keep |= (uint32_t)drop_keep(geo, (uint32_t)qcol.tok[acc_col(i)], c0 + (uint32_t)acc_row(i), sid) << i;
+    }
+    float s[32], dp[32];
+    sm90::wg_fence();
+#pragma unroll
+    for (int kk = 0; kk < HD / 16; ++kk) W64::ss(s, sm90::desc(Ks, HD, kk), sm90::desc(Qs, HD, kk), kk > 0);
+#pragma unroll
+    for (int kk = 0; kk < HD / 16; ++kk) W64::ss(dp, sm90::desc(Vs, HD, kk), sm90::desc(Gs, HD, kk), kk > 0);
+    sm90::wg_commit();
+    sm90::wg_wait0();
+    sm90::reg_fence(s);
+    sm90::reg_fence(dp);
+    if constexpr (DROP) {
 #pragma unroll
       for (int i = 0; i < 32; ++i) dp[i] = (keep >> i) & 1u ? dp[i] * geo.drop_scale : 0.f;
     }
     switch (epi) {
-      case 0: dkv_probs<false, 0>(s, dp, geo, qcol, tab, krow); break;
-      case 1: dkv_probs<false, 1>(s, dp, geo, qcol, tab, krow); break;
-      case 2: dkv_probs<false, 2>(s, dp, geo, qcol, tab, krow); break;
-      case 3: dkv_probs<true, 0>(s, dp, geo, qcol, tab, krow); break;
-      case 4: dkv_probs<true, 1>(s, dp, geo, qcol, tab, krow); break;
-      default: dkv_probs<true, 2>(s, dp, geo, qcol, tab, krow); break;
+      case 0: dkv_probs<false, 0>(s, dp, geo, qcol, tab, key_rows(geo, KR, KC, kpos)); break;
+      case 1: dkv_probs<false, 1>(s, dp, geo, qcol, tab, key_rows(geo, KR, KC, kpos)); break;
+      case 2: dkv_probs<false, 2>(s, dp, geo, qcol, tab, key_rows(geo, KR, KC, kpos)); break;
+      case 3: dkv_probs<true, 0>(s, dp, geo, qcol, tab, key_rows(geo, KR, KC, kpos)); break;
+      case 4: dkv_probs<true, 1>(s, dp, geo, qcol, tab, key_rows(geo, KR, KC, kpos)); break;
+      default: dkv_probs<true, 2>(s, dp, geo, qcol, tab, key_rows(geo, KR, KC, kpos)); break;
     }
     if constexpr (DROP) {
 #pragma unroll
@@ -654,14 +684,15 @@
     for (int kk = 0; kk < 4; ++kk) { to_a_frag<T>(s, kk, ap[kk]); to_a_frag<T>(dp, kk, ad[kk]); }
     sm90::wg_fence();
 #pragma unroll
-    for (int kk = 0; kk < 4; ++kk) WHD::rs(dvacc, ap[kk], sm90::desc(Gt, 64, kk), 1);
-#pragma unroll
-    for (int kk = 0; kk < 4; ++kk) WHD::rs(dkacc, ad[kk], sm90::desc(Qt, 64, kk), 1);
+    for (int kk = 0; kk < 4; ++kk) WHD::rs(dvacc, ap[kk], sm90::desc_mn(Gs, HD, kk), 1);
+#pragma unroll
+    for (int kk = 0; kk < 4; ++kk) WHD::rs(dkacc, ad[kk], sm90::desc_mn(Qs, HD, kk), 1);
     sm90::wg_commit();
     sm90::wg_wait0();
     sm90::reg_fence(dvacc);
     sm90::reg_fence(dkacc);
   }
+  const KRows krow = key_rows(geo, KR, KC, kpos);
 #pragma unroll
   for (int e = 0; e < 2; ++e) {
     if (!krow.real[e]) continue;
```

Result: faster. 3797, median of 6 (+4.5%).
